# cnkuangshi/LightCTR

Hardware: NVIDIA B200
Metric: samples/sec (device-timed) FM train step on Criteo-shape (higher is better)
Workload: dtype f32

## Files before the change

lightctr_b200/csrc/capi.cu:

```cuda
#include <stdarg.h>
#include <stdlib.h>
#include <string.h>

#include <algorithm>
#include <vector>

#include "opt.cuh"

namespace lctr {
static thread_local std::string g_err;
void set_error(const char* fmt, ...) {
    char buf[1024];
    va_list ap;
    va_start(ap, fmt);
    vsnprintf(buf, sizeof(buf), fmt, ap);
    va_end(ap);
    g_err = buf;
}

template <typename T>
static int dalloc(T** p, size_t n) {
    *p = nullptr;
    if (n == 0) return 0;
    LCTR_CUDA(cudaMalloc((void**)p, n * sizeof(T)));
    return 0;
}
template <typename T>
static void dfree(T*& p) {
    if (p) cudaFree(p);
    p = nullptr;
}

static int slot_reserve(lctr_ctx* c, Slot& s, int64_t rows, int64_t nnz) {
    const size_t k = c->cfg.factor_cnt;
    if (rows > s.cap_rows) {
        int64_t cap = std::max<int64_t>(rows, s.cap_rows + s.cap_rows / 2);
        dfree(s.row_ptr); dfree(s.label); dfree(s.pred); dfree(s.sumvx); dfree(s.wide);
        if (dalloc(&s.row_ptr, (size_t)cap + 1)) return 1;
        if (dalloc(&s.label, (size_t)cap)) return 1;
        if (dalloc(&s.pred, (size_t)cap)) return 1;
        if (dalloc(&s.wide, (size_t)cap)) return 1;
        if (c->cfg.model != LCTR_MODEL_FFM) {
            if (dalloc(&s.sumvx, (size_t)cap * k)) return 1;
            LCTR_CUDA(cudaMemsetAsync(s.sumvx, 0, (size_t)cap * k * sizeof(float), c->stream));
        }
        s.cap_rows = cap;
    }
    if (nnz > s.cap_nnz) {
        int64_t cap = std::max<int64_t>(nnz, s.cap_nnz + s.cap_nnz / 2);
        dfree(s.fid); dfree(s.field); dfree(s.val);
        if (dalloc(&s.fid, (size_t)cap + 32)) return 1;
        if (dalloc(&s.field, (size_t)cap + 32)) return 1;
        if (dalloc(&s.val, (size_t)cap + 32)) return 1;
        s.cap_nnz = cap;
    }
    return 0;
}

__global__ void fill_value_kernel(float* p, size_t n, float v) {
    for (size_t i = (size_t)blockIdx.x * blockDim.x + threadIdx.x; i < n; i += (size_t)gridDim.x * blockDim.x) p[i] = v;
}

__global__ void label_to_float_kernel(const int32_t* in, float* out, int64_t n_arg, const int64_t* hdr) {
    const int64_t n = hdr ? hdr[0] : n_arg;
    int64_t i = (int64_t)blockIdx.x * blockDim.x + threadIdx.x;
    if (i < n) out[i] = (float)in[i];
}

__global__ void fill_params_kernel(float* __restrict__ W, float* __restrict__ V, size_t Fl, size_t rowlen, int rank,
                                   int world, unsigned long long seed, float scale) {
    const size_t n = Fl * rowlen;
    for (size_t i = (size_t)blockIdx.x * blockDim.x + threadIdx.x; i < n; i += (size_t)gridDim.x * blockDim.x) {
        const size_t l = i / rowlen, j = i % rowlen;
        const unsigned long long g = ((unsigned long long)(l * world + rank)) * rowlen + j;
        unsigned long long h = g * 0x9E3779B97F4A7C15ull + seed;
        h ^= h >> 33; h *= 0xff51afd7ed558ccdull; h ^= h >> 33; h *= 0xc4ceb9fe1a85ec53ull; h ^= h >> 33;
        const float u1 = ((unsigned)(h & 0xffffffu) + 1u) * (1.0f / 16777217.0f);
        const float u2 = (unsigned)((h >> 24) & 0xffffffu) * (1.0f / 16777216.0f);
        V[i] = scale * sqrtf(-2.0f * logf(u1)) * cosf(6.2831853f * u2);
        if (j == 0) W[l] = 0.f;
    }
}

static int build_csc(lctr_ctx* c, Slot& s, int64_t rows, int64_t nnz, const int64_t* row_ptr, const uint32_t* fid,
                     const float* val) {
    const int64_t block = c->cfg.csc_row_block ? (int64_t)c->cfg.csc_row_block : std::max<int64_t>(rows, 1);
    const int64_t nblocks = (rows + block - 1) / block;
    std::vector<int64_t> blk_seg_ptr(nblocks + 1, 0), seg_ptr;
    std::vector<uint32_t> seg_fid, ent_row((size_t)nnz);
    std::vector<float> ent_x(val ? (size_t)nnz : 0);
    seg_ptr.reserve((size_t)nnz / 4 + 16);
    seg_fid.reserve((size_t)nnz / 4 + 16);
    std::vector<uint32_t> cnt(c->F + 1, 0);
    std::vector<uint32_t> touched_list;
    int64_t out = 0;
    for (int64_t bi = 0; bi < nblocks; bi++) {
        const int64_t rb = bi * block, re = std::min(rows, rb + block);
        const int64_t eb = row_ptr[rb], ee = row_ptr[re];
        touched_list.clear();
        for (int64_t e = eb; e < ee; e++) {
            const uint32_t f = fid[e];
            if (f >= c->F) { set_error("upload_batch: fid %u >= feature_cnt %zu", f, c->F); return 1; }
            if (cnt[f]++ == 0) touched_list.push_back(f);
        }
        std::sort(touched_list.begin(), touched_list.end());
        for (uint32_t f : touched_list) {
            seg_fid.push_back(f);
            seg_ptr.push_back(out);
            const uint32_t n = cnt[f];
            cnt[f] = (uint32_t)(out - eb);
            out += n;
        }
        for (int64_t r = rb; r < re; r++)
            for (int64_t e = row_ptr[r]; e < row_ptr[r + 1]; e++) {
                const uint32_t f = fid[e];
                const int64_t pos = eb + cnt[f]++;
                ent_row[(size_t)pos] = (uint32_t)r;
                if (val) ent_x[(size_t)pos] = val[e];
            }
        for (uint32_t f : touched_list) cnt[f] = 0;
        blk_seg_ptr[bi + 1] = (int64_t)seg_fid.size();
    }
    seg_ptr.push_back(out);
    const int64_t nseg = (int64_t)seg_fid.size();
    if (nseg > s.cap_segs) {
        dfree(s.seg_ptr); dfree(s.seg_fid);
        if (dalloc(&s.seg_ptr, (size_t)nseg + 1) || dalloc(&s.seg_fid, (size_t)nseg + 1)) return 1;
        s.cap_segs = nseg;
    }
    if (nblocks > s.cap_blocks) {
        dfree(s.blk_seg_ptr);
        if (dalloc(&s.blk_seg_ptr, (size_t)nblocks + 1)) return 1;
        s.cap_blocks = nblocks;
    }
    if (nnz > s.cap_ent) {
        dfree(s.ent_row); dfree(s.ent_x);
        if (dalloc(&s.ent_row, (size_t)nnz + 32) || dalloc(&s.ent_x, (size_t)nnz + 32)) return 1;
        s.cap_ent = nnz;
    }
    LCTR_CUDA(cudaMemcpyAsync(s.seg_ptr, seg_ptr.data(), (size_t)(nseg + 1) * sizeof(int64_t), cudaMemcpyHostToDevice, c->stream));
    if (nseg) LCTR_CUDA(cudaMemcpyAsync(s.seg_fid, seg_fid.data(), (size_t)nseg * sizeof(uint32_t), cudaMemcpyHostToDevice, c->stream));
    LCTR_CUDA(cudaMemcpyAsync(s.blk_seg_ptr, blk_seg_ptr.data(), (size_t)(nblocks + 1) * sizeof(int64_t), cudaMemcpyHostToDevice, c->stream));
    if (nnz) {
        LCTR_CUDA(cudaMemcpyAsync(s.ent_row, ent_row.data(), (size_t)nnz * sizeof(uint32_t), cudaMemcpyHostToDevice, c->stream));
        if (val) LCTR_CUDA(cudaMemcpyAsync(s.ent_x, ent_x.data(), (size_t)nnz * sizeof(float), cudaMemcpyHostToDevice, c->stream));
    }
    LCTR_CUDA(cudaStreamSynchronize(c->stream));
    if (!s.h_blk_seg_ptr) s.h_blk_seg_ptr = new std::vector<int64_t>();
    *s.h_blk_seg_ptr = blk_seg_ptr;
    s.csc_block = block; s.n_blocks = nblocks; s.n_segs = nseg;
    return 0;
}
}

using namespace lctr;

extern "C" {

const char* lctr_last_error(void) { return g_err.c_str(); }
int lctr_abi_version(void) { return LCTR_ABI_VERSION; }

int lctr_create(const lctr_cfg* cfg, lctr_ctx** out) {
    LCTR_CHECK(cfg && out, "lctr_create: null argument");
    LCTR_CHECK(cfg->abi_version == LCTR_ABI_VERSION, "lctr_create: abi_version %u != %u", cfg->abi_version,
               LCTR_ABI_VERSION);
    LCTR_CHECK(cfg->model >= LCTR_MODEL_FM && cfg->model <= LCTR_MODEL_WND, "lctr_create: bad model %d", cfg->model);
    LCTR_CHECK(cfg->optimizer >= LCTR_OPT_ADAGRAD && cfg->optimizer <= LCTR_OPT_PS_DCASGDA, "lctr_create: bad optimizer %d",
               cfg->optimizer);
    LCTR_CHECK(cfg->feature_cnt > 0 && cfg->feature_cnt < (1ull << 32), "lctr_create: feature_cnt out of range");
    LCTR_CHECK(cfg->factor_cnt > 0, "lctr_create: factor_cnt must be > 0");
    LCTR_CHECK(cfg->model != LCTR_MODEL_FFM || cfg->field_cnt > 0, "lctr_create: FFM needs field_cnt > 0");
    if (cfg->model == LCTR_MODEL_WND) {
        LCTR_CHECK(cfg->field_cnt > 0 && cfg->field_cnt <= 2048, "lctr_create: Wide&Deep needs 0 < field_cnt <= 2048");
        LCTR_CHECK(cfg->deterministic == 0, "lctr_create: Wide&Deep uses the RED scatter (deterministic = 0)");
    }
    int ndev = 0;
    cudaError_t e = cudaGetDeviceCount(&ndev);
    if (e != cudaSuccess || ndev == 0) {
        set_error("lctr_create: no CUDA device available (%s); this library has no CPU fallback",
                  cudaGetErrorString(e));
        return 2;
    }
    LCTR_CHECK(cfg->device >= 0 && cfg->device < ndev, "lctr_create: device %d of %d", cfg->device, ndev);
    LCTR_CUDA(cudaSetDevice(cfg->device));
    lctr_ctx* c = new lctr_ctx();
    c->cfg = *cfg;
    if (c->cfg.ftrl_alpha == 0.f) {
        c->cfg.ftrl_alpha = 0.15f; c->cfg.ftrl_lambda1 = 1.0f; c->cfg.ftrl_beta = 1.0f; c->cfg.ftrl_lambda2 = 1.0f;
    }
    if (c->cfg.world <= 0) { c->cfg.world = 1; c->cfg.rank = 0; }
    c->F = cfg->feature_cnt;
    c->Fl = (c->F + (size_t)c->cfg.world - 1) / (size_t)c->cfg.world;
    LCTR_CHECK(c->cfg.world == 1 || !cfg->deterministic, "lctr_create: deterministic modes are single-GPU only");
    LCTR_CHECK(cfg->deterministic >= 0 && cfg->deterministic <= 2, "lctr_create: deterministic must be 0, 1 or 2");
    c->rowlen = cfg->model == LCTR_MODEL_FFM ? (size_t)cfg->field_cnt * cfg->factor_cnt : cfg->factor_cnt;
    cudaDeviceProp prop;
    LCTR_CUDA(cudaGetDeviceProperties(&prop, cfg->device));
    c->sm_count = prop.multiProcessorCount;
    LCTR_CUDA(cudaStreamCreateWithFlags(&c->stream, cudaStreamNonBlocking));
    const size_t FL = c->Fl;
    const size_t nv = FL * c->rowlen;
    const bool two = cfg->optimizer == LCTR_OPT_FTRL || cfg->optimizer == LCTR_OPT_ADAM || cfg->optimizer == LCTR_OPT_ADADELTA ||
                     cfg->optimizer == LCTR_OPT_PS_DCASGD || cfg->optimizer == LCTR_OPT_PS_DCASGDA;
    int rc = 0;
    rc |= dalloc(&c->W, FL); rc |= dalloc(&c->V, nv);
    rc |= dalloc(&c->gW, FL); rc |= dalloc(&c->gV, nv);
    rc |= dalloc(&c->s1W, FL); rc |= dalloc(&c->s1V, nv);
    if (two) { rc |= dalloc(&c->s2W, FL); rc |= dalloc(&c->s2V, nv); }
    rc |= dalloc(&c->touched, FL + 512);
    rc |= dalloc(&c->touch_list, FL + 32);
    rc |= dalloc(&c->n_touch, 1);
    rc |= dalloc(&c->apply_done, 1);
    rc |= dalloc(&c->stats, (size_t)2 * kStatRing);
    rc |= dalloc(&c->stat_partial, 2);
    rc |= dalloc(&c->stat_done, 1);
    if (rc) { lctr_destroy(c); return 1; }
    LCTR_CUDA(cudaMallocHost((void**)&c->h_stats, 2 * sizeof(double)));
    LCTR_CUDA(cudaMemsetAsync(c->W, 0, FL * sizeof(float), c->stream));
    LCTR_CUDA(cudaMemsetAsync(c->V, 0, nv * sizeof(float), c->stream));
    LCTR_CUDA(cudaMemsetAsync(c->gW, 0, FL * sizeof(float), c->stream));
    LCTR_CUDA(cudaMemsetAsync(c->gV, 0, nv * sizeof(float), c->stream));
    LCTR_CUDA(cudaMemsetAsync(c->s1W, 0, FL * sizeof(float), c->stream));
    LCTR_CUDA(cudaMemsetAsync(c->s1V, 0, nv * sizeof(float), c->stream));
    if (two) {
        LCTR_CUDA(cudaMemsetAsync(c->s2W, 0, FL * sizeof(float), c->stream));
        LCTR_CUDA(cudaMemsetAsync(c->s2V, 0, nv * sizeof(float), c->stream));
    }
    if (cfg->optimizer == LCTR_OPT_PS_ADAGRAD || cfg->optimizer == LCTR_OPT_PS_DCASGDA) {
        fill_value_kernel<<<c->sm_count * 4, 256, 0, c->stream>>>(c->s1W, FL, 1e-7f);
        fill_value_kernel<<<c->sm_count * 4, 256, 0, c->stream>>>(c->s1V, nv, 1e-7f);
    }
    LCTR_CUDA(cudaMemsetAsync(c->touched, 0, FL + 512, c->stream));
    if (c->cfg.world > 1) {
        if (dist_alloc(c)) { lctr_destroy(c); return 1; }
    } else {
        c->cW = c->W; c->cV = c->V; c->cgW = c->gW; c->cgV = c->gV;
    }
    LCTR_CUDA(cudaMemsetAsync(c->n_touch, 0, sizeof(unsigned int), c->stream));
    LCTR_CUDA(cudaMemsetAsync(c->apply_done, 0, sizeof(unsigned int), c->stream));
    LCTR_CUDA(cudaMemsetAsync(c->stats, 0, sizeof(double) * 2 * kStatRing, c->stream));
    LCTR_CUDA(cudaMemsetAsync(c->stat_partial, 0, sizeof(double) * 2, c->stream));
    LCTR_CUDA(cudaMemsetAsync(c->stat_done, 0, sizeof(unsigned int), c->stream));
    if (cfg->model == LCTR_MODEL_NFM || cfg->model == LCTR_MODEL_WND) {
        if (mlp_alloc(c)) { lctr_destroy(c); return 1; }
    }
    { const char* e = getenv("LCTR_CSC_IN_STEP"); c->csc_in_step = e && e[0] == '1'; }
    LCTR_CUDA(cudaStreamSynchronize(c->stream));
    *out = c;
    return 0;
}

int lctr_destroy(lctr_ctx* c) {
    if (!c) return 0;
    cudaSetDevice(c->cfg.device);
    if (c->stream) cudaStreamSynchronize(c->stream);
    dfree(c->W); dfree(c->V); dfree(c->gW); dfree(c->gV); dfree(c->s1W); dfree(c->s1V); dfree(c->s2W); dfree(c->s2V);
    dfree(c->touched); dfree(c->touch_list); dfree(c->n_touch); dfree(c->apply_done); dfree(c->stats); dfree(c->stat_partial); dfree(c->stat_done);
    for (auto& s : c->slots) {
        dfree(s.row_ptr); dfree(s.fid); dfree(s.field); dfree(s.val); dfree(s.label); dfree(s.pred); dfree(s.sumvx);
        dfree(s.wide);
        dfree(s.blk_seg_ptr); dfree(s.seg_ptr); dfree(s.seg_fid); dfree(s.ent_row); dfree(s.ent_x); dfree(s.ent_field);
        dfree(s.ent_slot); dfree(s.ent_pslot); dfree(s.hot_of); dfree(s.hot_slot); dfree(s.n_hot);
        dfree(s.uniq); dfree(s.n_uniq); dfree(s.short_list); dfree(s.long_list); dfree(s.csc_totals); dfree(s.csc_acc); dfree(s.csc_arrived);
        delete s.h_blk_seg_ptr; s.h_blk_seg_ptr = nullptr;
    }
    mlp_free(c);
    ffm_grouped_free(c);
    metrics_free(c);
    wnd_free(c);
    dist_free(c);
    fused_free(c);
    csc_scratch_free(c);
    if (c->h_stats) cudaFreeHost(c->h_stats);
    if (c->h_stat_ring) cudaFreeHost(c->h_stat_ring);
    for (int p = 0; p < kPipe; p++) {
        PipeGraph& g = c->pipe_graph[p];
        if (g.build) cudaGraphExecDestroy(g.build);
        if (g.step) cudaGraphExecDestroy(g.step);
        if (g.d_hdr) cudaFree(g.d_hdr); if (g.h_hdr) cudaFreeHost(g.h_hdr);
        if (g.d_opt) cudaFree(g.d_opt); if (g.h_opt) cudaFreeHost(g.h_opt);
        if (g.d_stat) cudaFree(g.d_stat); if (g.h_stat) cudaFreeHost(g.h_stat);
    }
    if (c->copy_stream) {
        for (int i = 0; i < kPipe; i++) { cudaEventDestroy(c->ev_copied[i]); cudaEventDestroy(c->ev_computed[i]); cudaEventDestroy(c->ev_h2d[i]); }
        if (c->build_stream) cudaStreamDestroy(c->build_stream);
        for (int i = 0; i < kStatRing; i++) cudaEventDestroy(c->ev_stat[i]);
        cudaStreamDestroy(c->copy_stream);
    }
    if (c->stream) cudaStreamDestroy(c->stream);
    delete c;
    return 0;
}

int lctr_sync(lctr_ctx* c) {
    LCTR_CHECK(c, "null ctx");
    LCTR_CUDA(cudaStreamSynchronize(c->stream));
    return 0;
}

int lctr_upload_params(lctr_ctx* c, const float* W, const float* V) {
    LCTR_CHECK(c, "null ctx");
    const int R = c->cfg.world, me = c->cfg.rank;
    if (R == 1) {
        if (W) LCTR_CUDA(cudaMemcpyAsync(c->W, W, c->F * sizeof(float), cudaMemcpyHostToDevice, c->stream));
        if (V) LCTR_CUDA(cudaMemcpyAsync(c->V, V, c->F * c->rowlen * sizeof(float), cudaMemcpyHostToDevice, c->stream));
    } else {
        std::vector<float> w, v;
        if (W) {
            w.assign(c->Fl, 0.f);
            for (size_t f = (size_t)me, l = 0; f < c->F; f += R, l++) w[l] = W[f];
            LCTR_CUDA(cudaMemcpyAsync(c->W, w.data(), c->Fl * sizeof(float), cudaMemcpyHostToDevice, c->stream));
        }
        if (V) {
            v.assign(c->Fl * c->rowlen, 0.f);
            for (size_t f = (size_t)me, l = 0; f < c->F; f += R, l++)
                memcpy(&v[l * c->rowlen], V + f * c->rowlen, c->rowlen * sizeof(float));
            LCTR_CUDA(cudaMemcpyAsync(c->V, v.data(), v.size() * sizeof(float), cudaMemcpyHostToDevice, c->stream));
        }
        LCTR_CUDA(cudaStreamSynchronize(c->stream));
        return 0;
    }
    LCTR_CUDA(cudaStreamSynchronize(c->stream));
    return 0;
}
int lctr_download_params(lctr_ctx* c, float* W, float* V) {
    LCTR_CHECK(c, "null ctx");
    const int R = c->cfg.world, me = c->cfg.rank;
    if (R == 1) {
        if (W) LCTR_CUDA(cudaMemcpyAsync(W, c->W, c->F * sizeof(float), cudaMemcpyDeviceToHost, c->stream));
        if (V) LCTR_CUDA(cudaMemcpyAsync(V, c->V, c->F * c->rowlen * sizeof(float), cudaMemcpyDeviceToHost, c->stream));
        LCTR_CUDA(cudaStreamSynchronize(c->stream));
        return 0;
    }
    std::vector<float> w(c->Fl), v(c->Fl * c->rowlen);
    LCTR_CUDA(cudaMemcpyAsync(w.data(), c->W, w.size() * sizeof(float), cudaMemcpyDeviceToHost, c->stream));
    LCTR_CUDA(cudaMemcpyAsync(v.data(), c->V, v.size() * sizeof(float), cudaMemcpyDeviceToHost, c->stream));
    LCTR_CUDA(cudaStreamSynchronize(c->stream));
    for (size_t f = (size_t)me, l = 0; f < c->F; f += R, l++) {
        if (W) W[f] = w[l];
        if (V) memcpy(V + f * c->rowlen, &v[l * c->rowlen], c->rowlen * sizeof(float));
    }
    return 0;
}
int lctr_fill_params(lctr_ctx* c, uint64_t seed, float scale) {
    LCTR_CHECK(c, "null ctx");
    fill_params_kernel<<<c->sm_count * 8, 256, 0, c->stream>>>(c->W, c->V, c->Fl, c->rowlen, c->cfg.rank, c->cfg.world,
                                                               (unsigned long long)seed, scale);
    c->launches++;
    LCTR_CUDA(cudaGetLastError());
    LCTR_CUDA(cudaStreamSynchronize(c->stream));
    return 0;
}
int lctr_download_opt_state(lctr_ctx* c, float* s1, float* s2) {
    LCTR_CHECK(c, "null ctx");
    LCTR_CHECK(c->cfg.world == 1, "optimizer-state transfer is single-GPU only");
    const size_t nv = c->F * c->rowlen;
    if (s1) {
        LCTR_CUDA(cudaMemcpyAsync(s1, c->s1W, c->F * sizeof(float), cudaMemcpyDeviceToHost, c->stream));
        LCTR_CUDA(cudaMemcpyAsync(s1 + c->F, c->s1V, nv * sizeof(float), cudaMemcpyDeviceToHost, c->stream));
    }
    if (s2 && c->s2W) {
        LCTR_CUDA(cudaMemcpyAsync(s2, c->s2W, c->F * sizeof(float), cudaMemcpyDeviceToHost, c->stream));
        LCTR_CUDA(cudaMemcpyAsync(s2 + c->F, c->s2V, nv * sizeof(float), cudaMemcpyDeviceToHost, c->stream));
    }
    LCTR_CUDA(cudaStreamSynchronize(c->stream));
    return 0;
}
int lctr_upload_opt_state(lctr_ctx* c, const float* s1, const float* s2) {
    LCTR_CHECK(c, "null ctx");
    LCTR_CHECK(c->cfg.world == 1, "optimizer-state transfer is single-GPU only (the state arrays are sharded by owner)");
    const size_t nv = c->F * c->rowlen;
    if (s1) {
        LCTR_CUDA(cudaMemcpyAsync(c->s1W, s1, c->F * sizeof(float), cudaMemcpyHostToDevice, c->stream));
        LCTR_CUDA(cudaMemcpyAsync(c->s1V, s1 + c->F, nv * sizeof(float), cudaMemcpyHostToDevice, c->stream));
    }
    if (s2 && c->s2W) {
        LCTR_CUDA(cudaMemcpyAsync(c->s2W, s2, c->F * sizeof(float), cudaMemcpyHostToDevice, c->stream));
        LCTR_CUDA(cudaMemcpyAsync(c->s2V, s2 + c->F, nv * sizeof(float), cudaMemcpyHostToDevice, c->stream));
    }
    LCTR_CUDA(cudaStreamSynchronize(c->stream));
    return 0;
}

static int upload_batch_on(lctr_ctx* c, cudaStream_t st, int slot, int64_t rows, int64_t nnz, const int64_t* row_ptr,
                           const uint32_t* fid, const uint16_t* field, const float* val, const int32_t* label) {
    LCTR_CHECK(c, "null ctx");
    LCTR_CHECK(slot >= 0 && slot < kNumSlots, "slot %d out of range", slot);
    LCTR_CHECK(rows >= 0 && nnz >= 0 && row_ptr && (nnz == 0 || fid) && (rows == 0 || label), "upload_batch: null input");
    LCTR_CHECK((c->cfg.model != LCTR_MODEL_FFM && c->cfg.model != LCTR_MODEL_WND) || field || nnz == 0,
               "upload_batch: FFM / Wide&Deep need the field array");
    Slot& s = c->slots[slot];
    if (rows > s.cap_rows || nnz > s.cap_nnz) {
        LCTR_CUDA(cudaStreamSynchronize(c->stream));
        if (slot_reserve(c, s, rows, nnz)) return 1;
        LCTR_CUDA(cudaStreamSynchronize(c->stream));
    }
    s.rows = rows; s.nnz = nnz;
    s.has_val = val != nullptr;
    s.has_field = field != nullptr;
    LCTR_CUDA(cudaMemcpyAsync(s.row_ptr, row_ptr, (size_t)(rows + 1) * sizeof(int64_t), cudaMemcpyHostToDevice, st));
    if (nnz) {
        LCTR_CUDA(cudaMemcpyAsync(s.fid, fid, (size_t)nnz * sizeof(uint32_t), cudaMemcpyHostToDevice, st));
        if (field) LCTR_CUDA(cudaMemcpyAsync(s.field, field, (size_t)nnz * sizeof(uint16_t), cudaMemcpyHostToDevice, st));
        if (val) LCTR_CUDA(cudaMemcpyAsync(s.val, val, (size_t)nnz * sizeof(float), cudaMemcpyHostToDevice, st));
    }
    const bool grouped = c->cfg.deterministic == 2 && rows > 0 && nnz > 0 && c->cfg.world == 1;
    int32_t* tmp = reinterpret_cast<int32_t*>(s.pred);
    if (rows) {
        LCTR_CUDA(cudaMemcpyAsync(tmp, label, (size_t)rows * sizeof(int32_t), cudaMemcpyHostToDevice, st));
        if (!grouped) {
            label_to_float_kernel<<<(unsigned)((rows + 255) / 256), 256, 0, st>>>(tmp, s.label, rows, nullptr);
            c->launches++;
            LCTR_CUDA(cudaGetLastError());
        }
    }
    s.fused_valid = false;
    if ((fused_supported(c) || c->cfg.world > 1) && rows > 0 && nnz > 0) {
        if (fused_reserve(c, s, nnz) || fused_build_slot(c, s, st, nullptr, rows, nnz)) return 1;
        if (c->cfg.world > 1 && dist_send_keys(c, s, slot, st)) return 1;
    }
    s.csc_block = 0;
    s.dev_csc = false;
    if (grouped) {
        LCTR_CHECK(csc_device_supported(c), "cfg.deterministic=2 (device-grouped backward) needs FM with k in {4,8,16,32} "
                                            "or FFM with k %% 4 == 0 and field_cnt * k <= 512");
        if (csc_build_device(c, s, st, tmp, nullptr, rows, nnz)) return 1;
    } else if (c->cfg.deterministic == 1 && c->cfg.model != LCTR_MODEL_FFM && rows > 0) {
        LCTR_CUDA(cudaStreamSynchronize(st));
        if (build_csc(c, s, rows, nnz, row_ptr, fid, val)) return 1;
    }
    return 0;
}

int lctr_upload_batch(lctr_ctx* c, int slot, int64_t rows, int64_t nnz, const int64_t* row_ptr, const uint32_t* fid,
                      const uint16_t* field, const float* val, const int32_t* label) {
    LCTR_CHECK(c, "null ctx");
    LCTR_CHECK(rows >= 0 && nnz >= 0 && row_ptr && (nnz == 0 || fid), "upload_batch: null input");
    LCTR_CHECK(row_ptr[0] == 0 && row_ptr[rows] == nnz, "upload_batch: row_ptr must run from 0 to nnz (%lld .. %lld, nnz %lld)",
               (long long)row_ptr[0], (long long)row_ptr[rows], (long long)nnz);
    for (int64_t r = 0; r < rows; r++)
        LCTR_CHECK(row_ptr[r] <= row_ptr[r + 1], "upload_batch: row_ptr decreases at row %lld", (long long)r);
    for (int64_t i = 0; i < nnz; i++)
        LCTR_CHECK(fid[i] < c->F, "upload_batch: fid %u at entry %lld >= feature_cnt %zu", fid[i], (long long)i, c->F);
    if ((c->cfg.model == LCTR_MODEL_FFM || c->cfg.model == LCTR_MODEL_WND) && field)
        for (int64_t i = 0; i < nnz; i++)
            LCTR_CHECK(field[i] < c->cfg.field_cnt, "upload_batch: field %u at entry %lld >= field_cnt %u", (unsigned)field[i],
                       (long long)i, c->cfg.field_cnt);
    return upload_batch_on(c, c->stream, slot, rows, nnz, row_ptr, fid, field, val, label);
}

static int read_stats(lctr_ctx* c, uint64_t step, float* loss_sum, float* acc_cnt) {
    if (!loss_sum && !acc_cnt) return 0;
    if (c->cfg.world > 1 && dist_check_overflow(c)) return 1;
    LCTR_CUDA(cudaMemcpyAsync(c->h_stats, c->stats + 2 * (step % kStatRing), 2 * sizeof(double), cudaMemcpyDeviceToHost,
                              c->stream));
    LCTR_CUDA(cudaStreamSynchronize(c->stream));
    if (loss_sum) *loss_sum = (float)c->h_stats[0];
    if (acc_cnt) *acc_cnt = (float)c->h_stats[1];
    return 0;
}

int lctr_train_step(lctr_ctx* c, int slot, int64_t rb, int64_t re, float* loss_sum, float* acc_cnt) {
    LCTR_CHECK(c, "null ctx");
    LCTR_CHECK(slot >= 0 && slot < kNumSlots, "slot %d out of range", slot);
    Slot& s = c->slots[slot];
    LCTR_CHECK(rb >= 0 && re <= s.rows && rb <= re, "train_step: rows [%lld,%lld) outside slot (%lld rows)",
               (long long)rb, (long long)re, (long long)s.rows);
    LCTR_CHECK(c->cfg.world == 1 || c->cfg.minibatch_size > 0,
               "train_step: multi-GPU contexts need cfg.minibatch_size = the GLOBAL batch (the updater's divisor)");
    const uint64_t step = c->step;
    int rc = 0;
    if (c->csc_in_step && c->cfg.deterministic == 2 && c->cfg.world == 1 && rb == 0 && re == s.rows && s.nnz > 0) {
        ProfScope prof(c, PROF_CSC_BUILD);
        if (csc_build_device(c, s, c->stream, nullptr, nullptr, s.rows, s.nnz)) return 1;
    }
    switch (c->cfg.model) {
        case LCTR_MODEL_FM:
            if (c->cfg.world > 1 && fused_kernels_ok(c))
                rc = dist_pre_step(c, s, slot, true) || launch_fm_fused(c, s, rb, re, true, nullptr, nullptr) ||
                     dist_post_step(c, s, slot, re - rb);
            else if (c->cfg.world > 1)
                rc = dist_pre_step(c, s, slot, false) || launch_fm_forward(c, s, rb, re, false, true) ||
                     launch_fm_backward(c, s, rb, re, false) || dist_post_step(c, s, slot, re - rb);
            else if (c->cfg.deterministic == 2)
                rc = launch_fm_forward(c, s, rb, re, false, true) || launch_fm_backward_devcsc(c, s, rb, re);
            else if (c->cfg.deterministic)
                rc = launch_fm_forward(c, s, rb, re, false, true) || launch_fm_backward_csc(c, s, rb, re, false);
            else if (s.fused_valid)
                rc = launch_fm_fused(c, s, rb, re, true, nullptr, nullptr) || launch_apply_compact(c, s, re - rb, nullptr, nullptr);
            else
                rc = launch_fm_forward(c, s, rb, re, false, true) || launch_fm_backward(c, s, rb, re, false) ||
                     launch_apply(c, re - rb);
            break;
        case LCTR_MODEL_FFM:
            if (c->cfg.world > 1)
                rc = dist_pre_step(c, s, slot, false) || launch_ffm_forward(c, s, rb, re, true) || dist_post_step(c, s, slot, re - rb);
            else if (c->cfg.deterministic == 2)
                rc = ffm_grouped_reserve(c, s.rows) || launch_ffm_forward_tiles(c, s, rb, re) ||
                     launch_ffm_backward_grouped(c, s, rb, re);
            else
                rc = launch_ffm_forward(c, s, rb, re, true) || launch_ffm_backward(c, s, rb, re) || launch_apply(c, re - rb);
            break;
        case LCTR_MODEL_WND:
            if (c->cfg.world > 1)
                rc = dist_pre_step(c, s, slot, false) || mlp_reserve(c, re - rb) || wnd_reserve(c, re - rb) ||
                     launch_wnd_forward(c, s, rb, re) || launch_nfm_mlp(c, s, rb, re, re - rb) || launch_wnd_backward(c, s, rb, re) ||
                     dist_post_step(c, s, slot, re - rb);
            else
                rc = mlp_reserve(c, re - rb) || wnd_reserve(c, re - rb) || launch_wnd_forward(c, s, rb, re) ||
                     launch_nfm_mlp(c, s, rb, re, re - rb) || launch_wnd_backward(c, s, rb, re) || launch_apply(c, re - rb);
            break;
        case LCTR_MODEL_NFM:
            if (fused_kernels_ok(c) && s.fused_valid) {
                const bool multi = c->cfg.world > 1;
                rc = (multi && dist_pre_step(c, s, slot, true)) || mlp_reserve(c, re - rb) || launch_nfm_forward_fused(c, s, rb, re) ||
                     launch_nfm_mlp(c, s, rb, re, re - rb) || launch_nfm_backward_fused(c, s, rb, re) ||
                     (multi ? dist_post_step(c, s, slot, re - rb) : launch_apply_compact(c, s, re - rb, nullptr, nullptr));
                break;
            }
            if (c->cfg.world > 1) {
                rc = dist_pre_step(c, s, slot, false) || mlp_reserve(c, re - rb) || launch_fm_forward(c, s, rb, re, true, false) ||
                     launch_nfm_mlp(c, s, rb, re, re - rb) || launch_fm_backward(c, s, rb, re, true) ||
                     dist_post_step(c, s, slot, re - rb);
                break;
            }
            rc = mlp_reserve(c, re - rb) || launch_fm_forward(c, s, rb, re, true, false) ||
                 launch_nfm_mlp(c, s, rb, re, re - rb);
            if (!rc) {
                if (c->cfg.deterministic == 1) rc = launch_fm_backward_csc(c, s, rb, re, true);
                else rc = launch_fm_backward(c, s, rb, re, true) || launch_apply(c, re - rb);
            }
            break;
    }
    if (rc) return 1;
    c->step++;
    return read_stats(c, step, loss_sum, acc_cnt);
}

int lctr_train_batch(lctr_ctx* c, int64_t rows, int64_t nnz, const int64_t* row_ptr, const uint32_t* fid,
                     const uint16_t* field, const float* val, const int32_t* label, float* loss_sum, float* acc_cnt) {
    if (lctr_upload_batch(c, 0, rows, nnz, row_ptr, fid, field, val, label)) return 1;
    return lctr_train_step(c, 0, 0, rows, loss_sum, acc_cnt);
}

static int pipe_init(lctr_ctx* c) {
    if (c->copy_stream) return 0;
    LCTR_CUDA(cudaStreamCreateWithFlags(&c->copy_stream, cudaStreamNonBlocking));
    LCTR_CUDA(cudaStreamCreateWithFlags(&c->build_stream, cudaStreamNonBlocking));
    for (int i = 0; i < kPipe; i++) {
        LCTR_CUDA(cudaEventCreateWithFlags(&c->ev_copied[i], cudaEventDisableTiming));
        LCTR_CUDA(cudaEventCreateWithFlags(&c->ev_computed[i], cudaEventDisableTiming));
        LCTR_CUDA(cudaEventCreateWithFlags(&c->ev_h2d[i], cudaEventDisableTiming));
    }
    for (int i = 0; i < kStatRing; i++) LCTR_CUDA(cudaEventCreateWithFlags(&c->ev_stat[i], cudaEventDisableTiming));
    LCTR_CUDA(cudaMallocHost((void**)&c->h_stat_ring, sizeof(double) * 2 * kStatRing));
    return 0;
}

static int pipe_graph_capture(lctr_ctx* c, int p, bool has_val) {
    PipeGraph& g = c->pipe_graph[p];
    Slot& s = c->slots[kNumSlots - kPipe + p];
    if (g.build) { cudaGraphExecDestroy(g.build); g.build = nullptr; }
    if (g.step) { cudaGraphExecDestroy(g.step); g.step = nullptr; }
    if (!g.d_hdr) {
        LCTR_CUDA(cudaMalloc((void**)&g.d_hdr, 2 * sizeof(int64_t)));
        LCTR_CUDA(cudaMallocHost((void**)&g.h_hdr, 2 * sizeof(int64_t)));
        LCTR_CUDA(cudaMalloc((void**)&g.d_opt, csc_opt_params_size()));
        LCTR_CUDA(cudaMallocHost((void**)&g.h_opt, csc_opt_params_size()));
        LCTR_CUDA(cudaMalloc((void**)&g.d_stat, 2 * sizeof(double)));
        LCTR_CUDA(cudaMallocHost((void**)&g.h_stat, 2 * sizeof(double)));
    }
    s.has_val = has_val;
    {
        OptParams* hp = reinterpret_cast<OptParams*>(g.h_opt);
        memset(hp, 0, csc_opt_params_size());
        hp->opt = c->cfg.optimizer;
    }
    cudaGraph_t graph;
    const bool fused = fused_supported(c);
    LCTR_CUDA(cudaStreamBeginCapture(c->copy_stream, cudaStreamCaptureModeThreadLocal));
    int rc = cudaMemcpyAsync(g.d_hdr, g.h_hdr, 2 * sizeof(int64_t), cudaMemcpyHostToDevice, c->copy_stream) != cudaSuccess;
    if (!rc) {
        if (fused) {
            label_to_float_kernel<<<(unsigned)((s.cap_rows + 255) / 256), 256, 0, c->copy_stream>>>(
                reinterpret_cast<int32_t*>(s.pred), s.label, s.cap_rows, g.d_hdr);
            c->launches++;
            rc = fused_build_slot(c, s, c->copy_stream, g.d_hdr, s.cap_rows, s.cap_nnz);
        } else {
            rc = csc_build_device(c, s, c->copy_stream, reinterpret_cast<int32_t*>(s.pred), g.d_hdr, s.cap_rows, s.cap_nnz);
        }
    }
    cudaError_t ce = cudaStreamEndCapture(c->copy_stream, &graph);
    if (rc || ce != cudaSuccess) { set_error("streamed pipeline: capture of the build graph failed (%s)", cudaGetErrorString(ce)); return 1; }
    LCTR_CUDA(cudaGraphInstantiate(&g.build, graph, 0));
    cudaGraphDestroy(graph);
    LCTR_CUDA(cudaStreamBeginCapture(c->stream, cudaStreamCaptureModeThreadLocal));
    rc = cudaMemcpyAsync(g.d_opt, g.h_opt, csc_opt_params_size(), cudaMemcpyHostToDevice, c->stream) != cudaSuccess;
    if (!rc) {
        if (fused)
            rc = launch_fm_fused(c, s, 0, s.cap_rows, true, g.d_hdr, g.d_stat) ||
                 launch_apply_compact(c, s, s.cap_rows, reinterpret_cast<const OptParams*>(g.h_opt),
                                      reinterpret_cast<const OptParams*>(g.d_opt));
        else
            rc = launch_fm_forward_ex(c, s, 0, s.cap_rows, false, true, g.d_hdr, g.d_stat) ||
                 launch_fm_backward_devcsc_ex(c, s, 0, s.cap_rows, reinterpret_cast<const OptParams*>(g.h_opt), g.d_opt);
    }
    if (!rc) rc = cudaMemcpyAsync(g.h_stat, g.d_stat, 2 * sizeof(double), cudaMemcpyDeviceToHost, c->stream) != cudaSuccess;
    ce = cudaStreamEndCapture(c->stream, &graph);
    if (rc || ce != cudaSuccess) { set_error("streamed pipeline: capture of the step graph failed (%s)", cudaGetErrorString(ce)); return 1; }
    LCTR_CUDA(cudaGraphInstantiate(&g.step, graph, 0));
    cudaGraphDestroy(graph);
    g.cap_rows = s.cap_rows; g.cap_nnz = s.cap_nnz; g.has_val = has_val;
    return 0;
}

static int train_batch_async_graph(lctr_ctx* c, int64_t rows, int64_t nnz, const int64_t* row_ptr, const uint32_t* fid,
                                   const float* val, const int32_t* label, uint64_t* ticket) {
    const int p = (int)(c->pipe_issued % kPipe);
    const int slot = kNumSlots - kPipe + p;
    Slot& s = c->slots[slot];
    PipeGraph& g = c->pipe_graph[p];
    if (rows > s.cap_rows || nnz > s.cap_nnz || !g.build || g.has_val != (val != nullptr) || g.cap_rows != s.cap_rows ||
        g.cap_nnz != s.cap_nnz) {
        LCTR_CUDA(cudaStreamSynchronize(c->stream));
        LCTR_CUDA(cudaStreamSynchronize(c->copy_stream));
        LCTR_CUDA(cudaStreamSynchronize(c->build_stream));
        if (rows > s.cap_rows || nnz > s.cap_nnz)
            if (slot_reserve(c, s, std::max(rows, s.cap_rows) + rows / 8 + 64, std::max(nnz, s.cap_nnz) + nnz / 8 + 1024)) return 1;
        if (fused_supported(c) ? fused_reserve(c, s, s.cap_nnz) : csc_reserve(c, s, s.cap_nnz)) return 1;
        LCTR_CUDA(cudaStreamSynchronize(c->stream));
        if (pipe_graph_capture(c, p, val != nullptr)) return 1;
    }
    s.rows = rows; s.nnz = nnz; s.has_val = val != nullptr; s.has_field = false;
    if (c->pipe_issued >= (uint64_t)kPipe) LCTR_CUDA(cudaStreamWaitEvent(c->copy_stream, c->ev_computed[p], 0));
    LCTR_CUDA(cudaMemcpyAsync(s.row_ptr, row_ptr, (size_t)(rows + 1) * sizeof(int64_t), cudaMemcpyHostToDevice, c->copy_stream));
    LCTR_CUDA(cudaMemcpyAsync(s.fid, fid, (size_t)nnz * sizeof(uint32_t), cudaMemcpyHostToDevice, c->copy_stream));
    if (val) LCTR_CUDA(cudaMemcpyAsync(s.val, val, (size_t)nnz * sizeof(float), cudaMemcpyHostToDevice, c->copy_stream));
    LCTR_CUDA(cudaMemcpyAsync(s.pred, label, (size_t)rows * sizeof(int32_t), cudaMemcpyHostToDevice, c->copy_stream));
    g.h_hdr[0] = rows; g.h_hdr[1] = nnz;
    LCTR_CUDA(cudaEventRecord(c->ev_h2d[p], c->copy_stream));
    LCTR_CUDA(cudaStreamWaitEvent(c->build_stream, c->ev_h2d[p], 0));
    LCTR_CUDA(cudaGraphLaunch(g.build, c->build_stream));
    LCTR_CUDA(cudaEventRecord(c->ev_copied[p], c->build_stream));
    LCTR_CUDA(cudaStreamWaitEvent(c->stream, c->ev_copied[p], 0));
    const bool fused = fused_supported(c);
    if (fused) fused_opt_params(c, rows, g.h_opt); else csc_opt_params(c, rows, g.h_opt);
    LCTR_CUDA(cudaGraphLaunch(g.step, c->stream));
    LCTR_CUDA(cudaEventRecord(c->ev_computed[p], c->stream));
    s.dev_csc = !fused;
    s.fused_valid = fused;
    c->launches += 8;
    g.ticket = c->step;
    *ticket = c->step++;
    c->pipe_issued++;
    return 0;
}

int lctr_train_batch_async(lctr_ctx* c, int64_t rows, int64_t nnz, const int64_t* row_ptr, const uint32_t* fid,
                           const uint16_t* field, const float* val, const int32_t* label, uint64_t* ticket) {
    LCTR_CHECK(c && ticket, "null argument");
    LCTR_CHECK(c->cfg.deterministic != 1, "streamed batches need cfg.deterministic 0 (RED scatter) or 2 (device grouping)");
    if (pipe_init(c)) return 1;
    LCTR_CHECK(c->pipe_issued - c->pipe_waited < (uint64_t)kPipe, "more than %d streamed batches outstanding: call lctr_wait first", kPipe);
    if ((c->cfg.deterministic == 2 || fused_supported(c)) && c->cfg.world == 1 && c->cfg.model == LCTR_MODEL_FM && !c->profiling &&
        rows > 0 && nnz > 0)
        return train_batch_async_graph(c, rows, nnz, row_ptr, fid, val, label, ticket);
    const int p = (int)(c->pipe_issued % kPipe);
    const int slot = kNumSlots - kPipe + p;
    if (c->pipe_issued >= (uint64_t)kPipe) LCTR_CUDA(cudaStreamWaitEvent(c->copy_stream, c->ev_computed[p], 0));
    if (c->pipe_issued >= 1) LCTR_CUDA(cudaStreamWaitEvent(c->copy_stream, c->ev_copied[(p + kPipe - 1) % kPipe], 0));
    if (upload_batch_on(c, c->copy_stream, slot, rows, nnz, row_ptr, fid, field, val, label)) return 1;
    LCTR_CUDA(cudaEventRecord(c->ev_copied[p], c->copy_stream));
    LCTR_CUDA(cudaStreamWaitEvent(c->stream, c->ev_copied[p], 0));
    const uint64_t step = c->step;
    if (lctr_train_step(c, slot, 0, rows, nullptr, nullptr)) return 1;
    LCTR_CUDA(cudaEventRecord(c->ev_computed[p], c->stream));
    const int ri = (int)(step % kStatRing);
    LCTR_CUDA(cudaMemcpyAsync(c->h_stat_ring + 2 * ri, c->stats + 2 * ri, 2 * sizeof(double), cudaMemcpyDeviceToHost, c->stream));
    LCTR_CUDA(cudaEventRecord(c->ev_stat[ri], c->stream));
    c->pipe_graph[p].ticket = ~0ull;
    *ticket = step;
    c->pipe_issued++;
    return 0;
}

int lctr_wait(lctr_ctx* c, uint64_t ticket, float* loss_sum, float* acc_cnt) {
    LCTR_CHECK(c && c->copy_stream, "lctr_wait: no streamed batch was issued");
    LCTR_CHECK(ticket < c->step && c->step - ticket <= (uint64_t)kStatRing, "lctr_wait: ticket %llu is not outstanding",
               (unsigned long long)ticket);
    for (int p = 0; p < kPipe; p++) {
        if (c->pipe_graph[p].build && c->pipe_graph[p].ticket == ticket) {
            LCTR_CUDA(cudaEventSynchronize(c->ev_computed[p]));
            if (loss_sum) *loss_sum = (float)c->pipe_graph[p].h_stat[0];
            if (acc_cnt) *acc_cnt = (float)c->pipe_graph[p].h_stat[1];
            if (c->pipe_waited < c->pipe_issued) c->pipe_waited++;
            return 0;
        }
    }
    const int ri = (int)(ticket % kStatRing);
    LCTR_CUDA(cudaEventSynchronize(c->ev_stat[ri]));
    if (loss_sum) *loss_sum = (float)c->h_stat_ring[2 * ri];
    if (acc_cnt) *acc_cnt = (float)c->h_stat_ring[2 * ri + 1];
    if (c->pipe_waited < c->pipe_issued) c->pipe_waited++;
    return 0;
}

int lctr_predict(lctr_ctx* c, int slot, int quirk_sumvx_slot, float* pctr) {
    LCTR_CHECK(c, "null ctx");
    LCTR_CHECK(slot >= 0 && slot < kNumSlots, "slot %d out of range", slot);
    Slot& s = c->slots[slot];
    int rc = 0;
    if (c->cfg.model == LCTR_MODEL_WND) {
        const float* out = nullptr;
        rc = (c->cfg.world > 1 && dist_pre_step(c, s, slot, false)) || mlp_reserve(c, s.rows) || wnd_reserve(c, s.rows) ||
             launch_wnd_forward(c, s, 0, s.rows) || mlp_forward_only(c, s.rows, &out) || launch_wnd_pred(c, s, out, 0, s.rows);
        if (rc) return 1;
        if (pctr) {
            LCTR_CUDA(cudaMemcpyAsync(pctr, s.pred, (size_t)s.rows * sizeof(float), cudaMemcpyDeviceToHost, c->stream));
            LCTR_CUDA(cudaStreamSynchronize(c->stream));
        }
        return 0;
    }
    LCTR_CHECK(c->cfg.world == 1, "lctr_predict: multi-GPU contexts keep sharded tables; download the parameters "
                                  "(lctr_download_params) into a single-GPU context to predict");
    if (c->cfg.model == LCTR_MODEL_FFM) {
        rc = c->cfg.deterministic == 1 ? launch_ffm_predict_inorder(c, s) : launch_ffm_forward(c, s, 0, s.rows, false);
    } else if (c->cfg.model == LCTR_MODEL_FM) {
        if (quirk_sumvx_slot >= 0) {
            LCTR_CHECK(quirk_sumvx_slot < kNumSlots, "quirk slot out of range");
            rc = launch_predict_quirk(c, s, c->slots[quirk_sumvx_slot]);
        } else {
            rc = fused_supported(c) ? launch_fm_forward_tree(c, s, 0, s.rows, false) : launch_fm_forward(c, s, 0, s.rows, false, false);
        }
    } else {
        set_error("lctr_predict: the reference ships no NFM predictor (main.cpp:230-233)");
        return 1;
    }
    if (rc) return 1;
    if (pctr) {
        LCTR_CUDA(cudaMemcpyAsync(pctr, s.pred, (size_t)s.rows * sizeof(float), cudaMemcpyDeviceToHost, c->stream));
        LCTR_CUDA(cudaStreamSynchronize(c->stream));
    }
    return 0;
}

int lctr_download_sumvx(lctr_ctx* c, int slot, float* out) {
    LCTR_CHECK(c && out, "null argument");
    LCTR_CHECK(slot >= 0 && slot < kNumSlots, "slot %d out of range", slot);
    Slot& s = c->slots[slot];
    LCTR_CHECK(s.sumvx, "model has no sumVX (FFM keeps it NULL, fm_predict.cpp:20)");
    LCTR_CUDA(cudaMemcpyAsync(out, s.sumvx, (size_t)s.rows * c->cfg.factor_cnt * sizeof(float), cudaMemcpyDeviceToHost,
                              c->stream));
    LCTR_CUDA(cudaStreamSynchronize(c->stream));
    return 0;
}
int lctr_download_pred(lctr_ctx* c, int slot, float* out) {
    LCTR_CHECK(c && out, "null argument");
    LCTR_CHECK(slot >= 0 && slot < kNumSlots, "slot %d out of range", slot);
    Slot& s = c->slots[slot];
    LCTR_CUDA(cudaMemcpyAsync(out, s.pred, (size_t)s.rows * sizeof(float), cudaMemcpyDeviceToHost, c->stream));
    LCTR_CUDA(cudaStreamSynchronize(c->stream));
    return 0;
}

int lctr_dense_grad_buffer(lctr_ctx* c, void** dev_ptr, size_t* n_floats) {
    LCTR_CHECK(c && dev_ptr && n_floats, "null argument");
    *dev_ptr = c->dense_grad;
    *n_floats = c->dense_grad_n;
    return 0;
}

int lctr_profile(lctr_ctx* c, int enable) {
    LCTR_CHECK(c, "null ctx");
    if (enable && !c->prof_ev) { c->prof_ev = new std::vector<cudaEvent_t>(); c->prof_id = new std::vector<int>(); }
    c->profiling = enable ? 1 : 0;
    return 0;
}
int lctr_profile_read(lctr_ctx* c, double* ms, int64_t* counts, int n, int reset) {
    LCTR_CHECK(c && ms && counts, "null argument");
    LCTR_CUDA(cudaStreamSynchronize(c->stream));
    if (c->prof_ev) {
        for (size_t i = 0; i < c->prof_id->size(); i++) {
            float t = 0.f;
            cudaEventElapsedTime(&t, (*c->prof_ev)[2 * i], (*c->prof_ev)[2 * i + 1]);
            const int id = (*c->prof_id)[i];
            if (id >= 0 && id < kNumProf) { c->prof_ms[id] += t; c->prof_cnt[id]++; }
            cudaEventDestroy((*c->prof_ev)[2 * i]); cudaEventDestroy((*c->prof_ev)[2 * i + 1]);
        }
        c->prof_ev->clear(); c->prof_id->clear();
    }
    for (int i = 0; i < n && i < kNumProf; i++) { ms[i] = c->prof_ms[i]; counts[i] = c->prof_cnt[i]; }
    if (reset) for (int i = 0; i < kNumProf; i++) { c->prof_ms[i] = 0; c->prof_cnt[i] = 0; }
    return 0;
}

int64_t lctr_launch_count(const lctr_ctx* c) { return c ? c->launches : 0; }
void* lctr_stream(lctr_ctx* c) { return c ? (void*)c->stream : nullptr; }

}
```

lightctr_b200/csrc/common.cuh:

```cuda
#pragma once
#include <cuda_runtime.h>
#include <stdint.h>
#include <stdio.h>
#include <string>
#include <vector>

#include "../../include/lightctr_b200.h"
#include "ref_expf.h"

namespace lctr {

void set_error(const char* fmt, ...);

#define LCTR_CUDA(call)                                                                         \
    do {                                                                                        \
        cudaError_t _e = (call);                                                                \
        if (_e != cudaSuccess) {                                                                \
            ::lctr::set_error("%s:%d: %s -> %s", __FILE__, __LINE__, #call, cudaGetErrorString(_e)); \
            return 1;                                                                           \
        }                                                                                       \
    } while (0)

#define LCTR_CHECK(cond, ...)                  \
    do {                                       \
        if (!(cond)) {                         \
            ::lctr::set_error(__VA_ARGS__);    \
            return 1;                          \
        }                                      \
    } while (0)

constexpr int kNumSlots = 8;
constexpr int kPipe = LCTR_PIPE_DEPTH;
constexpr int kNumProf = 16;
enum { PROF_FM_FWD = 0, PROF_FM_BWD_RED = 1, PROF_APPLY = 2, PROF_FFM_FUSED = 3, PROF_FM_BWD_CSC = 4, PROF_MLP = 5, PROF_DIST_MARK = 6, PROF_DIST_COMPACT = 7, PROF_DIST_PULL = 8, PROF_DIST_PUSH = 9, PROF_DIST_BAR0 = 10, PROF_DIST_MERGE = 11, PROF_DIST_BAR1 = 12, PROF_CSC_BUILD = 13, PROF_FM_FUSED = 14, PROF_APPLY_COMPACT = 15 };
constexpr int kStatRing = 64;
constexpr int kHotRep = 32;
constexpr int kHotMax = 2048;
constexpr uint32_t kHotBit = 0x80000000u;
constexpr unsigned kFull = 0xffffffffu;

struct Slot {
    int64_t rows = 0, nnz = 0, cap_rows = 0, cap_nnz = 0;
    int64_t* row_ptr = nullptr;
    uint32_t* fid = nullptr;
    uint16_t* field = nullptr;
    float* val = nullptr;
    float* label = nullptr;
    float* pred = nullptr;
    float* sumvx = nullptr;
    float* wide = nullptr;
    bool has_val = false, has_field = false;
    int64_t csc_block = 0;
    int64_t n_blocks = 0, n_segs = 0;
    int64_t* blk_seg_ptr = nullptr;
    int64_t* seg_ptr = nullptr;
    uint32_t* seg_fid = nullptr;
    uint32_t* ent_row = nullptr;
    float* ent_x = nullptr;
    uint16_t* ent_field = nullptr;
    std::vector<int64_t>* h_blk_seg_ptr = nullptr;
    int64_t cap_segs = 0, cap_blocks = 0, cap_ent = 0;
    bool dev_csc = false;
    uint32_t *short_list = nullptr, *long_list = nullptr;
    int64_t cap_long = 0;
    double* csc_acc = nullptr;
    unsigned int* csc_arrived = nullptr;
    unsigned int* csc_totals = nullptr;
    uint32_t* uniq = nullptr;
    unsigned int* n_uniq = nullptr;
    int64_t cap_uniq = 0;
    bool uniq_valid = false;
    uint32_t* ent_slot = nullptr;
    uint32_t* ent_pslot = nullptr;
    int64_t cap_ent_slot = 0;
    uint32_t *hot_of = nullptr, *hot_slot = nullptr;
    unsigned int* n_hot = nullptr;
    bool fused_valid = false;
};

struct PipeGraph {
    cudaGraphExec_t build = nullptr, step = nullptr;
    int64_t cap_rows = 0, cap_nnz = 0;
    bool has_val = false;
    int64_t *d_hdr = nullptr, *h_hdr = nullptr;
    void *d_opt = nullptr, *h_opt = nullptr;
    double *d_stat = nullptr, *h_stat = nullptr;
    uint64_t ticket = ~0ull;
};

struct MlpLayer {
    int in = 0, out = 0;
    float *w = nullptr, *b = nullptr, *mask = nullptr;
    float *dw = nullptr, *db = nullptr;
    float *acc_w = nullptr, *acc_b = nullptr;
    float* act = nullptr;
    float* delta = nullptr;
    void* w16 = nullptr;
    void* w16t = nullptr;
};

}

namespace lctr {
struct DistState;
struct OptParams;
struct FusedState {
    uint8_t* mark = nullptr;
    size_t T = 0;
    uint32_t* slot_of = nullptr;
    unsigned int* cnt = nullptr;
    size_t cnt_cap = 0;
    float* G = nullptr;
    size_t G_rows = 0;
    float* Ghot = nullptr;
    OptParams* d_opt = nullptr;
    int GS = 0;
};
}
struct lctr_ctx {
    lctr_cfg cfg;
    cudaStream_t stream = nullptr;
    size_t F = 0, rowlen = 0;
    size_t Fl = 0;
    float *W = nullptr, *V = nullptr, *gW = nullptr, *gV = nullptr;
    float *s1W = nullptr, *s1V = nullptr, *s2W = nullptr, *s2V = nullptr;
    uint8_t* touched = nullptr;
    float *cW = nullptr, *cV = nullptr, *cgW = nullptr, *cgV = nullptr;
    lctr::DistState* dist = nullptr;
    lctr::FusedState* fused = nullptr;
    size_t dist_rows = 0;
    uint32_t* touch_list = nullptr;
    unsigned int* n_touch = nullptr;
    unsigned int* apply_done = nullptr;
    double* stats = nullptr;
    double* stat_partial = nullptr;
    unsigned int* stat_done = nullptr;
    double* h_stats = nullptr;
    uint64_t step = 0;
    size_t adam_iter = 0;
    lctr::Slot slots[lctr::kNumSlots];
    int n_layers = 0;
    lctr::MlpLayer layers[LCTR_MAX_LAYERS + 1];
    float* dense_grad = nullptr;
    size_t dense_grad_n = 0;
    float *z = nullptr, *dz = nullptr;
    float* mlp_out = nullptr;
    size_t mlp_cap_rows = 0;
    int64_t mlp_fwd_rows = 0;
    uint32_t* wnd_src = nullptr;
    size_t wnd_cap_rows = 0;
    void* auc_scratch = nullptr;
    int csc_in_step = 0;
    float* ffm_T = nullptr;
    uint16_t* ffm_cnt = nullptr;
    size_t ffm_T_rows = 0;
    lctr_allreduce_fn dense_allreduce = nullptr;
    void* dense_allreduce_user = nullptr;
    int mlp_tm = 0;
    size_t mlp_smem = 0;
    int mlp_umma = 0;
    size_t mlp_umma_smem = 0;
    int mlp_has_mask = 0;
    int mlp_skip_update = 0;
    int sm_count = 148;
    int64_t launches = 0;
    const unsigned long long* apply_wait_flags = nullptr;
    int apply_wait_n = 0;
    unsigned long long apply_wait_epoch = 0;
    const float* fwd_quirk_sumvx = nullptr;
    int64_t fwd_quirk_rows = 0;
    void* csc_scratch = nullptr;
    int profiling = 0;
    std::vector<cudaEvent_t>* prof_ev = nullptr;
    std::vector<int>* prof_id = nullptr;
    double prof_ms[lctr::kNumProf] = {0};
    int64_t prof_cnt[lctr::kNumProf] = {0};
    cudaStream_t copy_stream = nullptr;
    cudaEvent_t ev_copied[lctr::kPipe] = {}, ev_computed[lctr::kPipe] = {};
    cudaStream_t build_stream = nullptr;
    cudaEvent_t ev_h2d[lctr::kPipe] = {};
    cudaEvent_t ev_stat[lctr::kStatRing] = {nullptr};
    double* h_stat_ring = nullptr;
    uint64_t pipe_issued = 0, pipe_waited = 0;
    lctr::PipeGraph pipe_graph[lctr::kPipe];
};

namespace lctr {

__device__ __forceinline__ float warp_sum(float v) {
#pragma unroll
    for (int o = 16; o > 0; o >>= 1) v += __shfl_xor_sync(kFull, v, o);
    return v;
}
__device__ __forceinline__ double warp_sum_d(double v) {
#pragma unroll
    for (int o = 16; o > 0; o >>= 1) v += __shfl_xor_sync(kFull, v, o);
    return v;
}
__device__ __forceinline__ void red_add_v4(float* addr, float4 v) {
    asm volatile("red.global.add.v4.f32 [%0], {%1, %2, %3, %4};" ::"l"(addr), "f"(v.x), "f"(v.y), "f"(v.z), "f"(v.w)
                 : "memory");
}
__device__ __forceinline__ void red_add_f32(float* addr, float v) {
    asm volatile("red.global.add.f32 [%0], %1;" ::"l"(addr), "f"(v) : "memory");
}
__device__ __forceinline__ float4 ldg_f4(const float* p) { return __ldg(reinterpret_cast<const float4*>(p)); }
__device__ __forceinline__ float4 ldg_f4_pinned(const float* p) {
    float4 v;
    asm volatile("ld.global.nc.v4.f32 {%0,%1,%2,%3}, [%4];" : "=f"(v.x), "=f"(v.y), "=f"(v.z), "=f"(v.w) : "l"(p));
    return v;
}
__device__ __forceinline__ float ldg_f32_pinned(const float* p) {
    float v;
    asm volatile("ld.global.nc.f32 %0, [%1];" : "=f"(v) : "l"(p));
    return v;
}

template <typename FX, typename FY>
__device__ __forceinline__ float avx_dot_seq(FX x, FY y, int n) {
    float result = 0.f;
    int i = 0;
    if (n > 7) {
        float d[8] = {0.f, 0.f, 0.f, 0.f, 0.f, 0.f, 0.f, 0.f};
        for (; i + 8 <= n; i += 8) {
#pragma unroll
            for (int l = 0; l < 8; l++) d[l] = d[l] + x(i + l) * y(i + l);
        }
        const float a0 = d[4] + d[0], a1 = d[5] + d[1], a2 = d[6] + d[2], a3 = d[7] + d[3];
        const float b0 = a0 + a2, b1 = a1 + a3;
        result = result + (b0 + b1);
    }
    for (; i < n; i++) result = result + x(i) * y(i);
    return result;
}

__device__ __forceinline__ float ref_sigmoid(float x) {
    if (x < -16.f) return 1e-7f;
    if (x > 16.f) return 0.99999988f;
    return 1.0f / (1.0f + lctr_ref_expf(-x));
}
__device__ __forceinline__ float ref_exp_any(float x) { return fabsf(x) < 87.f ? lctr_ref_expf(x) : expf(x); }
__device__ __forceinline__ void loss_terms(float p, float y, double& loss, double& correct) {
    loss = (y == 1.f) ? (double)(-logf(p)) : -log(1.0 - (double)p);
    correct = ((p > 0.5f && y == 1.f) || (p < 0.5f && y == 0.f)) ? 1.0 : 0.0;
}

__device__ __forceinline__ void publish_stats(double loss, double correct, double* partial, unsigned int* done,
                                               double* out_slot, bool accumulate_out) {
    __shared__ double sh[2][32];
    const int lane = threadIdx.x & 31, wid = threadIdx.x >> 5, nw = (blockDim.x + 31) >> 5;
    loss = warp_sum_d(loss);
    correct = warp_sum_d(correct);
    if (lane == 0) { sh[0][wid] = loss; sh[1][wid] = correct; }
    __syncthreads();
    if (wid == 0) {
        double a = lane < nw ? sh[0][lane] : 0.0, b = lane < nw ? sh[1][lane] : 0.0;
        a = warp_sum_d(a);
        b = warp_sum_d(b);
        if (lane == 0) {
            atomicAdd(&partial[0], a);
            atomicAdd(&partial[1], b);
            __threadfence();
            unsigned int prev = atomicAdd(done, 1u);
            if (prev == gridDim.x - 1) {
                __threadfence();
                double l = atomicAdd(&partial[0], 0.0), c = atomicAdd(&partial[1], 0.0);
                if (accumulate_out) { out_slot[0] += l; out_slot[1] += c; }
                else { out_slot[0] = l; out_slot[1] = c; }
                partial[0] = 0.0; partial[1] = 0.0;
                *done = 0u;
                __threadfence();
            }
        }
    }
}

struct ProfScope {
    lctr_ctx* c; int id; cudaEvent_t a = nullptr, b = nullptr;
    ProfScope(lctr_ctx* c_, int id_) : c(c_), id(id_) {
        if (!c->profiling) return;
        cudaEventCreate(&a); cudaEventCreate(&b);
        cudaEventRecord(a, c->stream);
    }
    ~ProfScope() {
        if (!a) return;
        cudaEventRecord(b, c->stream);
        c->prof_ev->push_back(a); c->prof_ev->push_back(b); c->prof_id->push_back(id);
    }
};
int launch_fm_forward(lctr_ctx* c, Slot& s, int64_t rb, int64_t re, bool nfm, bool stats);
int launch_fm_backward(lctr_ctx* c, Slot& s, int64_t rb, int64_t re, bool nfm);
int launch_ffm_forward(lctr_ctx* c, Slot& s, int64_t rb, int64_t re, bool stats);
int launch_ffm_backward(lctr_ctx* c, Slot& s, int64_t rb, int64_t re);
int launch_apply(lctr_ctx* c, int64_t rows_in_step);
int launch_fm_backward_csc(lctr_ctx* c, Slot& s, int64_t rb, int64_t re, bool nfm);
int csc_reserve(lctr_ctx* c, Slot& s, int64_t max_nnz);
int csc_build_device(lctr_ctx* c, Slot& s, cudaStream_t st, const int32_t* label_i32, const int64_t* hdr,
                     int64_t rows_cap, int64_t nnz_cap);
int launch_fm_backward_devcsc(lctr_ctx* c, Slot& s, int64_t rb, int64_t re);
struct OptParams;
int launch_fm_backward_devcsc_ex(lctr_ctx* c, Slot& s, int64_t rb, int64_t re, const OptParams* P_host, const void* dP);
void csc_opt_params(lctr_ctx* c, int64_t rows, void* out);
size_t csc_opt_params_size();
int launch_fm_forward_ex(lctr_ctx* c, Slot& s, int64_t rb, int64_t re, bool nfm, bool stats, const int64_t* hdr,
                         double* out_slot_override);
bool csc_device_supported(const lctr_ctx* c);
void csc_scratch_free(lctr_ctx* c);
int launch_predict_quirk(lctr_ctx* c, Slot& s, Slot& train);
bool fused_supported(const lctr_ctx* c);
bool fused_kernels_ok(const lctr_ctx* c);
void fused_free(lctr_ctx* c);
int fused_reserve(lctr_ctx* c, Slot& s, int64_t nnz);
int fused_build_slot(lctr_ctx* c, Slot& s, cudaStream_t st, const int64_t* hdr, int64_t rows_cap, int64_t nnz_cap);
void dist_wait_info(lctr_ctx* c, const unsigned long long** flags, int* n, unsigned long long* epoch);
int launch_fm_fused(lctr_ctx* c, Slot& s, int64_t rb, int64_t re, bool stats, const int64_t* hdr, double* out_slot_override);
int launch_fm_forward_tree(lctr_ctx* c, Slot& s, int64_t rb, int64_t re, bool stats);
int launch_nfm_forward_fused(lctr_ctx* c, Slot& s, int64_t rb, int64_t re);
int launch_nfm_backward_fused(lctr_ctx* c, Slot& s, int64_t rb, int64_t re);
int launch_apply_compact(lctr_ctx* c, Slot& s, int64_t rows_in_step, const OptParams* P_host, const OptParams* dP);
void fused_opt_params(lctr_ctx* c, int64_t rows, void* out);
void* fused_dev_opt(lctr_ctx* c);
int launch_ffm_predict_inorder(lctr_ctx* c, Slot& s);
int dist_alloc(lctr_ctx* c);
int dist_free(lctr_ctx* c);
int dist_send_keys(lctr_ctx* c, Slot& s, int slot, cudaStream_t st);
int dist_pre_step(lctr_ctx* c, Slot& s, int slot, bool in_kernel_wait);
int dist_post_step(lctr_ctx* c, Slot& s, int slot, int64_t rows_divisor);
int dist_check_overflow(lctr_ctx* c);
size_t dist_bytes(const lctr_ctx* c);
__global__ void compact_touched_kernel(uint8_t* touched, size_t F, uint32_t* list, unsigned int* n_list,
                                       const unsigned long long* wait_flags, int n_wait, unsigned long long wait_epoch);
int mlp_alloc(lctr_ctx* c);
int mlp_free(lctr_ctx* c);
int mlp_reserve(lctr_ctx* c, int64_t rows);
bool ffm_grouped_supported(const lctr_ctx* c);
int ffm_grouped_reserve(lctr_ctx* c, int64_t rows);
void ffm_grouped_free(lctr_ctx* c);
int launch_ffm_forward_tiles(lctr_ctx* c, Slot& s, int64_t rb, int64_t re);
int launch_ffm_backward_grouped(lctr_ctx* c, Slot& s, int64_t rb, int64_t re);
void metrics_free(lctr_ctx* c);
int wnd_reserve(lctr_ctx* c, int64_t rows);
void wnd_free(lctr_ctx* c);
int launch_wnd_forward(lctr_ctx* c, Slot& s, int64_t rb, int64_t re);
int launch_wnd_backward(lctr_ctx* c, Slot& s, int64_t rb, int64_t re);
int launch_wnd_pred(lctr_ctx* c, Slot& s, const float* mlp_out, int64_t rb, int64_t re);
int mlp_forward_only(lctr_ctx* c, int64_t rows, const float** out);
inline size_t mlp_in0(const lctr_cfg& cf) {
    return cf.model == LCTR_MODEL_WND ? (size_t)cf.field_cnt * cf.factor_cnt : (size_t)cf.factor_cnt;
}
int mlp_sync_dense_grad(lctr_ctx* c);
bool pdl_on();
void launch_slotmap_compact(lctr_ctx* c, uint8_t* mark, size_t T, uint32_t* uniq, unsigned int* n_uniq, cudaStream_t st);
int launch_ffm_warp(lctr_ctx* c, Slot& s, int64_t rb, int64_t re, bool stats);
int mlp_bf16_prepare(lctr_ctx* c);
int mlp_bf16_refresh(lctr_ctx* c, int layer);
int launch_nfm_mlp_bf16(lctr_ctx* c, Slot& s, int64_t rb, int64_t re, int64_t rows_divisor);
int launch_nfm_mlp(lctr_ctx* c, Slot& s, int64_t rb, int64_t re, int64_t rows_divisor);

}
```

lightctr_b200/csrc/fm_fused.cu:

```cuda
#include <algorithm>

#include "fm_fused.cuh"

namespace lctr {

bool fused_kernels_ok(const lctr_ctx* c) {
    const int k = (int)c->cfg.factor_cnt;
    return (c->cfg.model == LCTR_MODEL_FM || c->cfg.model == LCTR_MODEL_NFM) && c->cfg.deterministic == 0 &&
           (k == 4 || k == 8 || k == 16 || k == 32);
}
bool fused_supported(const lctr_ctx* c) { return c->cfg.world == 1 && fused_kernels_ok(c); }

void fused_free(lctr_ctx* c) {
    FusedState* f = c->fused;
    if (!f) return;
    cudaFree(f->mark); cudaFree(f->slot_of); cudaFree(f->cnt); cudaFree(f->G); cudaFree(f->Ghot); cudaFree(f->d_opt);
    delete f;
    c->fused = nullptr;
}

static int fused_init(lctr_ctx* c) {
    if (c->fused) return 0;
    FusedState* f = new FusedState();
    c->fused = f;
    f->T = mark_rows(c->F);
    f->GS = fused_kernels_ok(c) ? grad_stride((int)c->cfg.factor_cnt) : 0;
    LCTR_CUDA(cudaMalloc((void**)&f->mark, 128 * f->T + 512));
    LCTR_CUDA(cudaMemsetAsync(f->mark, 0, 128 * f->T + 512, c->stream));
    LCTR_CUDA(cudaMalloc((void**)&f->slot_of, c->F * sizeof(uint32_t)));
    if (f->GS) {
        LCTR_CUDA(cudaMalloc((void**)&f->Ghot, (size_t)kHotMax * kHotRep * f->GS * sizeof(float)));
        LCTR_CUDA(cudaMemsetAsync(f->Ghot, 0, (size_t)kHotMax * kHotRep * f->GS * sizeof(float), c->stream));
    }
    LCTR_CUDA(cudaMalloc((void**)&f->d_opt, sizeof(OptParams)));
    LCTR_CUDA(cudaStreamSynchronize(c->stream));
    return 0;
}

int fused_reserve(lctr_ctx* c, Slot& s, int64_t nnz) {
    if (fused_init(c)) return 1;
    FusedState* f = c->fused;
    const int64_t need_u = std::min<int64_t>(std::max<int64_t>(nnz, 1), (int64_t)c->F);
    if (nnz > s.cap_ent_slot) {
        LCTR_CUDA(cudaStreamSynchronize(c->stream));
        if (s.ent_slot) cudaFree(s.ent_slot);
        if (s.ent_pslot) cudaFree(s.ent_pslot);
        s.ent_pslot = nullptr;
        const int64_t cap = std::max<int64_t>(nnz, s.cap_ent_slot + s.cap_ent_slot / 2);
        LCTR_CUDA(cudaMalloc((void**)&s.ent_slot, (size_t)(cap + 64) * sizeof(uint32_t)));
        if (c->cfg.world > 1) LCTR_CUDA(cudaMalloc((void**)&s.ent_pslot, (size_t)(cap + 64) * sizeof(uint32_t)));
        s.cap_ent_slot = cap;
    }
    if (need_u > s.cap_uniq || !s.hot_of) {
        LCTR_CUDA(cudaStreamSynchronize(c->stream));
        if (s.uniq) cudaFree(s.uniq);
        if (s.hot_of) cudaFree(s.hot_of);
        const int64_t cap = std::min<int64_t>(std::max<int64_t>(need_u, s.cap_uniq + s.cap_uniq / 2), (int64_t)c->F);
        LCTR_CUDA(cudaMalloc((void**)&s.uniq, (size_t)(cap + 64) * sizeof(uint32_t)));
        LCTR_CUDA(cudaMalloc((void**)&s.hot_of, (size_t)(cap + 64) * sizeof(uint32_t)));
        if (!s.n_uniq) LCTR_CUDA(cudaMalloc((void**)&s.n_uniq, sizeof(unsigned int)));
        if (!s.n_hot) LCTR_CUDA(cudaMalloc((void**)&s.n_hot, sizeof(unsigned int)));
        if (!s.hot_slot) LCTR_CUDA(cudaMalloc((void**)&s.hot_slot, (size_t)kHotMax * sizeof(uint32_t)));
        s.cap_uniq = cap;
    }
    if ((size_t)s.cap_uniq > f->cnt_cap) {
        LCTR_CUDA(cudaStreamSynchronize(c->stream));
        if (c->copy_stream) LCTR_CUDA(cudaStreamSynchronize(c->copy_stream));
        if (f->cnt) cudaFree(f->cnt);
        LCTR_CUDA(cudaMalloc((void**)&f->cnt, (size_t)(s.cap_uniq + 64) * sizeof(unsigned int)));
        LCTR_CUDA(cudaMemset(f->cnt, 0, (size_t)(s.cap_uniq + 64) * sizeof(unsigned int)));
        f->cnt_cap = (size_t)s.cap_uniq;
    }
    const size_t g_rows = c->cfg.world > 1 ? c->dist_rows : (size_t)s.cap_uniq;
    if (f->GS && g_rows > f->G_rows) {
        LCTR_CUDA(cudaStreamSynchronize(c->stream));
        if (f->G) cudaFree(f->G);
        LCTR_CUDA(cudaMalloc((void**)&f->G, (g_rows + 64) * f->GS * sizeof(float)));
        LCTR_CUDA(cudaMemset(f->G, 0, (g_rows + 64) * f->GS * sizeof(float)));
        f->G_rows = g_rows;
    }
    return 0;
}

int fused_build_slot(lctr_ctx* c, Slot& s, cudaStream_t st, const int64_t* hdr, int64_t rows_cap, int64_t nnz_cap) {
    FusedState* f = c->fused;
    s.fused_valid = false;
    if (rows_cap <= 0 || nnz_cap <= 0) return 0;
    const int SM = c->sm_count;
    LCTR_CUDA(cudaMemsetAsync(s.n_uniq, 0, sizeof(unsigned int), st));
    LCTR_CUDA(cudaMemsetAsync(s.n_hot, 0, sizeof(unsigned int), st));
    const unsigned mkg = (unsigned)std::max<int64_t>(1, std::min<int64_t>((nnz_cap + 2047) / 2048, (int64_t)SM * 4));
    slotmap_mark_kernel<<<mkg, 256, 0, st>>>(s.fid, hdr, nnz_cap, f->mark, f->T);
    const size_t ntiles = (128 * f->T + 511) / 512;
    const unsigned cg = (unsigned)std::max<size_t>(1, std::min<size_t>((ntiles + 7) / 8, (size_t)SM * 8));
    slotmap_compact_kernel<<<cg, 256, 0, st>>>(f->mark, f->T, s.uniq, s.n_uniq, f->slot_of);
    const bool hot = f->GS != 0;
    if (hot) {
        const unsigned sg = (unsigned)std::min<int64_t>(((int64_t)kHotSampleRows * 128 + 255) / 256, (int64_t)SM * 8);
        slotmap_sample_kernel<<<sg, 256, 0, st>>>(s.row_ptr, s.fid, hdr, rows_cap, f->slot_of, f->cnt);
        slotmap_hot_kernel<<<SM * 2, 256, 0, st>>>(f->cnt, s.n_uniq, hdr, rows_cap, s.hot_of, s.hot_slot, s.n_hot);
        c->launches += 2;
    }
    const unsigned ag = (unsigned)std::max<int64_t>(1, std::min<int64_t>((nnz_cap + 255) / 256, (int64_t)SM * 8));
    slotmap_assign_kernel<<<ag, 256, 0, st>>>(s.fid, hdr, nnz_cap, f->slot_of, hot ? s.hot_of : nullptr, s.ent_slot,
                                              c->cfg.world > 1 ? s.ent_pslot : nullptr);
    c->launches += 3;
    LCTR_CUDA(cudaGetLastError());
    s.fused_valid = true;
    return 0;
}

void launch_slotmap_compact(lctr_ctx* c, uint8_t* mark, size_t T, uint32_t* uniq, unsigned int* n_uniq, cudaStream_t st) {
    const size_t ntiles = (128 * T + 511) / 512;
    const unsigned cg = (unsigned)std::max<size_t>(1, std::min<size_t>((ntiles + 7) / 8, (size_t)c->sm_count * 8));
    slotmap_compact_kernel<<<cg, 256, 0, st>>>(mark, T, uniq, n_uniq, nullptr);
}

bool pdl_on() {
    const char* e = getenv("LCTR_PDL");
    return !(e && atoi(e) == 0);
}

template <int K>
static void fused_go(lctr_ctx* c, Slot& s, int64_t rb, int64_t re, int stats, double* out_slot, const int64_t* hdr, int mode) {
    FusedState* f = c->fused;
    const unsigned grid = (unsigned)std::max<int64_t>(1, std::min<int64_t>((re - rb + 3) / 4, (int64_t)c->sm_count * 4));
    const bool multi = c->cfg.world > 1;
    const unsigned long long* wf = nullptr;
    int nw = 0;
    unsigned long long ep = 0;
    if (multi && mode != 3) dist_wait_info(c, &wf, &nw, &ep);
#define FUSED_ARGS s.row_ptr, multi ? s.ent_pslot : s.fid, s.ent_slot, s.val, s.label, c->cW, c->cV, s.pred, s.sumvx, nullptr, f->G, \
                   f->Ghot, f->GS, c->cfg.l2_reg, rb, re, hdr, c->stat_partial, c->stat_done, out_slot, stats, wf, nw, ep
#define FUSED_LAUNCH(HV)                                                                                                         \
    do {                                                                                                                         \
        if (mode == 1 && multi && pdl_on()) {   \
            cudaLaunchConfig_t cfg = {};                                                                                         \
            cfg.gridDim = dim3(grid); cfg.blockDim = dim3(128); cfg.stream = c->stream;                                          \
            cudaLaunchAttribute at[1];                                                                                           \
            at[0].id = cudaLaunchAttributeProgrammaticStreamSerialization;                                                       \
            at[0].val.programmaticStreamSerializationAllowed = 1;                                                                \
            cfg.attrs = at; cfg.numAttrs = 1;                                                                                    \
            cudaLaunchKernelEx(&cfg, fm_fused_kernel<K, HV, 1, false>, (const int64_t*)s.row_ptr, (const uint32_t*)s.ent_pslot,  \
                               (const uint32_t*)s.ent_slot, (const float*)s.val, (const float*)s.label, (const float*)c->cW,   \
                               (const float*)c->cV, s.pred, s.sumvx, (float*)nullptr, f->G, f->Ghot, f->GS, c->cfg.l2_reg, rb, re, hdr, \
                               c->stat_partial, c->stat_done, out_slot, stats, wf, nw, ep, (float*)nullptr, (float*)nullptr);    \
        } else if (mode == 1) fm_fused_kernel<K, HV, 1, false><<<grid, 128, 0, c->stream>>>(FUSED_ARGS);                         \
        else if (mode == 2) fm_fused_kernel<K, HV, 2, false><<<grid, 128, 0, c->stream>>>(FUSED_ARGS, c->z, s.wide);             \
        else {   \
            cudaLaunchConfig_t cfg = {};                                                                                         \
            cfg.gridDim = dim3(grid); cfg.blockDim = dim3(128); cfg.stream = c->stream;                                          \
            cudaLaunchAttribute at[1];                                                                                           \
            at[0].id = cudaLaunchAttributeProgrammaticStreamSerialization;                                                       \
            at[0].val.programmaticStreamSerializationAllowed = 1;                                                                \
            cfg.attrs = at; cfg.numAttrs = (!multi && pdl_on()) ? 1 : 0;                                                         \
            cudaLaunchKernelEx(&cfg, fm_fused_kernel<K, HV, 3, false>, (const int64_t*)s.row_ptr, (const uint32_t*)(multi ? s.ent_pslot : s.fid), \
                               (const uint32_t*)s.ent_slot, (const float*)s.val, (const float*)s.label, (const float*)c->cW,   \
                               (const float*)c->cV, s.pred, s.sumvx, (float*)nullptr, f->G, f->Ghot, f->GS, c->cfg.l2_reg, rb, re, hdr, \
                               c->stat_partial, c->stat_done, out_slot, stats, wf, nw, ep, c->dz, (float*)nullptr);              \
        }                                                                                                                        \
    } while (0)
    if (s.has_val) FUSED_LAUNCH(true); else FUSED_LAUNCH(false);
#undef FUSED_LAUNCH
#undef FUSED_ARGS
}

static int launch_fused_mode(lctr_ctx* c, Slot& s, int64_t rb, int64_t re, bool stats, const int64_t* hdr, double* out_slot_override,
                             int mode, int prof_id) {
    if (re - rb <= 0) return 0;
    LCTR_CHECK(s.fused_valid, "fused FM step on a slot without its slot map (uploaded before the context supported it?)");
    double* out_slot = out_slot_override ? out_slot_override : c->stats + 2 * (c->step % kStatRing);
    ProfScope prof(c, prof_id);
    switch ((int)c->cfg.factor_cnt) {
        case 4: fused_go<4>(c, s, rb, re, stats ? 1 : 0, out_slot, hdr, mode); break;
        case 8: fused_go<8>(c, s, rb, re, stats ? 1 : 0, out_slot, hdr, mode); break;
        case 16: fused_go<16>(c, s, rb, re, stats ? 1 : 0, out_slot, hdr, mode); break;
        default: fused_go<32>(c, s, rb, re, stats ? 1 : 0, out_slot, hdr, mode); break;
    }
    c->launches++;
    LCTR_CUDA(cudaGetLastError());
    return 0;
}

int launch_fm_fused(lctr_ctx* c, Slot& s, int64_t rb, int64_t re, bool stats, const int64_t* hdr, double* out_slot_override) {
    return launch_fused_mode(c, s, rb, re, stats, hdr, out_slot_override, 1, PROF_FM_FUSED);
}
int launch_nfm_forward_fused(lctr_ctx* c, Slot& s, int64_t rb, int64_t re) {
    return launch_fused_mode(c, s, rb, re, false, nullptr, nullptr, 2, PROF_FM_FWD);
}
int launch_nfm_backward_fused(lctr_ctx* c, Slot& s, int64_t rb, int64_t re) {
    return launch_fused_mode(c, s, rb, re, false, nullptr, nullptr, 3, PROF_FM_FUSED);
}

template <int K>
static void fwd_tree_go(lctr_ctx* c, Slot& s, int64_t rb, int64_t re, int stats, double* out_slot) {
    const int GS = grad_stride(K);
    const unsigned grid = (unsigned)std::max<int64_t>(1, std::min<int64_t>((re - rb + 3) / 4, (int64_t)c->sm_count * 4));
#define FWD_ARGS s.row_ptr, s.fid, s.fid, s.val, s.label, c->W, c->V, s.pred, s.sumvx, nullptr, nullptr, nullptr, GS, c->cfg.l2_reg, \
                 rb, re, nullptr, c->stat_partial, c->stat_done, out_slot, stats
    if (s.has_val) fm_fused_kernel<K, true, 0, true><<<grid, 128, 0, c->stream>>>(FWD_ARGS);
    else fm_fused_kernel<K, false, 0, true><<<grid, 128, 0, c->stream>>>(FWD_ARGS);
#undef FWD_ARGS
}
int launch_fm_forward_tree(lctr_ctx* c, Slot& s, int64_t rb, int64_t re, bool stats) {
    if (re - rb <= 0) return 0;
    double* out_slot = c->stats + 2 * (c->step % kStatRing);
    ProfScope prof(c, PROF_FM_FWD);
    switch ((int)c->cfg.factor_cnt) {
        case 4: fwd_tree_go<4>(c, s, rb, re, stats ? 1 : 0, out_slot); break;
        case 8: fwd_tree_go<8>(c, s, rb, re, stats ? 1 : 0, out_slot); break;
        case 16: fwd_tree_go<16>(c, s, rb, re, stats ? 1 : 0, out_slot); break;
        default: fwd_tree_go<32>(c, s, rb, re, stats ? 1 : 0, out_slot); break;
    }
    c->launches++;
    LCTR_CUDA(cudaGetLastError());
    return 0;
}

template <int K>
static void apply_go(lctr_ctx* c, Slot& s, const OptParams& P, const OptParams* P_dev) {
    FusedState* f = c->fused;
    const int main_blocks = c->sm_count * 3;
    const unsigned grid = (unsigned)(main_blocks + kHotMax / 8);
    const bool pdl_off = !pdl_on();
    cudaLaunchConfig_t cfg = {};
    cfg.gridDim = dim3(grid); cfg.blockDim = dim3(256); cfg.dynamicSmemBytes = 0; cfg.stream = c->stream;
    cudaLaunchAttribute attr[1];
    attr[0].id = cudaLaunchAttributeProgrammaticStreamSerialization;
    attr[0].val.programmaticStreamSerializationAllowed = 1;
    cfg.attrs = attr;
    cfg.numAttrs = (c->cfg.world == 1 && !pdl_off) ? 1 : 0;
#define AC_GO(OPTC)                                                                                                          \
    cudaLaunchKernelEx(&cfg, apply_compact_kernel<K, OPTC>, (const uint32_t*)s.uniq, (const unsigned int*)s.n_uniq, f->G,          \
                       (const uint32_t*)s.hot_of, (const uint32_t*)s.hot_slot, (const unsigned int*)s.n_hot, f->Ghot, f->GS,     \
                       main_blocks, c->W, c->V, c->s1W, c->s1V, c->s2W, c->s2V, P, P_dev)
    switch (P.opt) {
        case LCTR_OPT_ADAGRAD: AC_GO(LCTR_OPT_ADAGRAD); break;
        case LCTR_OPT_FTRL: AC_GO(LCTR_OPT_FTRL); break;
        case LCTR_OPT_ADAM: AC_GO(LCTR_OPT_ADAM); break;
        case LCTR_OPT_RMSPROP: AC_GO(LCTR_OPT_RMSPROP); break;
        case LCTR_OPT_ADADELTA: AC_GO(LCTR_OPT_ADADELTA); break;
        case LCTR_OPT_PS_SGD: AC_GO(LCTR_OPT_PS_SGD); break;
        case LCTR_OPT_PS_ADAGRAD: AC_GO(LCTR_OPT_PS_ADAGRAD); break;
        case LCTR_OPT_PS_DCASGD: AC_GO(LCTR_OPT_PS_DCASGD); break;
        default: AC_GO(LCTR_OPT_PS_DCASGDA); break;
    }
#undef AC_GO
}

int launch_apply_compact(lctr_ctx* c, Slot& s, int64_t rows_in_step, const OptParams* P_host, const OptParams* dP) {
    const OptParams P = P_host ? *P_host : make_opt_params(c, rows_in_step);
    ProfScope prof(c, PROF_APPLY_COMPACT);
    switch ((int)c->cfg.factor_cnt) {
        case 4: apply_go<4>(c, s, P, dP); break;
        case 8: apply_go<8>(c, s, P, dP); break;
        case 16: apply_go<16>(c, s, P, dP); break;
        default: apply_go<32>(c, s, P, dP); break;
    }
    c->launches++;
    LCTR_CUDA(cudaGetLastError());
    return 0;
}

void fused_opt_params(lctr_ctx* c, int64_t rows, void* out) { *reinterpret_cast<OptParams*>(out) = make_opt_params(c, rows); }
void* fused_dev_opt(lctr_ctx* c) { return c->fused ? (void*)c->fused->d_opt : nullptr; }

}
```

lightctr_b200/csrc/fm_fused.cuh:

```cuda
#pragma once
#include "opt.cuh"

namespace lctr {

constexpr int kHotSampleRows = 512;
__host__ __device__ constexpr int grad_stride(int k) { return k < 8 ? 8 : (k < 16 ? 16 : (k < 32 ? 32 : 64)); }

__device__ __forceinline__ uint32_t ldg_u32_pinned(const uint32_t* p) {
    uint32_t v;
    asm volatile("ld.global.nc.u32 %0, [%1];" : "=r"(v) : "l"(p));
    return v;
}

constexpr int kMarkTags = 2048;
__host__ __device__ inline size_t mark_rows(size_t F) { return (F + 127) / 128; }
__global__ void __launch_bounds__(256)
slotmap_mark_kernel(const uint32_t* __restrict__ fid, const int64_t* __restrict__ hdr, int64_t nnz_arg,
                    uint8_t* __restrict__ mark, size_t T) {
    __shared__ uint32_t tag[kMarkTags];
    const int64_t nnz = hdr ? hdr[1] : nnz_arg;
    for (int i = threadIdx.x; i < kMarkTags; i += blockDim.x) tag[i] = 0xffffffffu;
    __syncthreads();
    const int64_t per = (nnz + gridDim.x - 1) / gridDim.x;
    const int64_t b = (int64_t)blockIdx.x * per, e = min(nnz, b + per);
    for (int64_t i0 = b + threadIdx.x; i0 < e; i0 += 4 * blockDim.x) {
        uint32_t f[4];
#pragma unroll
        for (int u = 0; u < 4; u++) {
            const int64_t i = i0 + (int64_t)u * blockDim.x;
            f[u] = i < e ? ldg_u32_pinned(fid + i) : 0xffffffffu;
        }
#pragma unroll
        for (int u = 0; u < 4; u++) {
            if (f[u] == 0xffffffffu) continue;
            const uint32_t h = f[u] & (kMarkTags - 1);
            if (tag[h] != f[u]) {
                tag[h] = f[u];
                mark[(size_t)(f[u] & 127u) * T + (f[u] >> 7)] = 1;
            }
        }
    }
}

__global__ void __launch_bounds__(256)
slotmap_compact_kernel(uint8_t* __restrict__ mark, size_t T, uint32_t* __restrict__ uniq, unsigned int* __restrict__ n_uniq,
                       uint32_t* __restrict__ slot_of) {
    const size_t F = 128 * T;
    const int lane = threadIdx.x & 31;
    const size_t warp = (size_t)blockIdx.x * (blockDim.x >> 5) + (threadIdx.x >> 5);
    const size_t nwarps = (size_t)gridDim.x * (blockDim.x >> 5);
    const size_t ntiles = (F + 511) / 512;
    for (size_t tile = warp; tile < ntiles; tile += nwarps) {
        const size_t base = tile * 512 + (size_t)lane * 16;
        uint4 m = make_uint4(0, 0, 0, 0);
        if (base + 16 <= F) {
            m = *reinterpret_cast<const uint4*>(mark + base);
        } else if (base < F) {
            unsigned char tmp[16];
            for (int i = 0; i < 16; i++) tmp[i] = base + i < F ? mark[base + i] : 0;
            m = *reinterpret_cast<uint4*>(tmp);
        }
        const bool any = (m.x | m.y | m.z | m.w) != 0;
        if (!__any_sync(kFull, any)) continue;
        unsigned bits = 0;
        {
            const unsigned wv[4] = {m.x, m.y, m.z, m.w};
#pragma unroll
            for (int i = 0; i < 4; i++)
#pragma unroll
                for (int b = 0; b < 4; b++)
                    if ((wv[i] >> (8 * b)) & 0xffu) bits |= 1u << (i * 4 + b);
        }
        if (any) {
            if (base + 16 <= F) *reinterpret_cast<uint4*>(mark + base) = make_uint4(0, 0, 0, 0);
            else for (int i = 0; i < 16 && base + i < F; i++) mark[base + i] = 0;
        }
        const int mycnt = __popc(bits);
        int incl = mycnt;
#pragma unroll
        for (int o = 1; o < 32; o <<= 1) {
            const int t = __shfl_up_sync(kFull, incl, o);
            if (lane >= o) incl += t;
        }
        const int total = __shfl_sync(kFull, incl, 31);
        unsigned int gbase = 0;
        if (lane == 31) gbase = atomicAdd(n_uniq, (unsigned int)total);
        gbase = __shfl_sync(kFull, gbase, 31);
        unsigned int pos = gbase + (unsigned int)(incl - mycnt);
        while (bits) {
            const int bit = __ffs(bits) - 1;
            bits &= bits - 1;
            const size_t ps = base + bit;
            const uint32_t f = (uint32_t)(((ps % T) << 7) | (ps / T));
            uniq[pos] = f;
            if (slot_of) slot_of[f] = pos;
            pos++;
        }
    }
}

__global__ void __launch_bounds__(256)
slotmap_sample_kernel(const int64_t* __restrict__ row_ptr, const uint32_t* __restrict__ fid, const int64_t* __restrict__ hdr,
                      int64_t rows_arg, const uint32_t* __restrict__ slot_of, unsigned int* __restrict__ cnt) {
    const int64_t rows = hdr ? hdr[0] : rows_arg;
    const int64_t ns = row_ptr[rows < kHotSampleRows ? rows : kHotSampleRows];
    for (int64_t i = (int64_t)blockIdx.x * blockDim.x + threadIdx.x; i < ns; i += (int64_t)gridDim.x * blockDim.x)
        atomicAdd(&cnt[slot_of[fid[i]]], 1u);
}

__global__ void __launch_bounds__(256)
slotmap_hot_kernel(unsigned int* __restrict__ cnt, const unsigned int* __restrict__ n_uniq, const int64_t* __restrict__ hdr,
                   int64_t rows_arg, uint32_t* __restrict__ hot_of, uint32_t* __restrict__ hot_slot,
                   unsigned int* __restrict__ n_hot) {
    const int64_t rows = hdr ? hdr[0] : rows_arg;
    const int64_t srows = rows < kHotSampleRows ? rows : kHotSampleRows;
    const unsigned thr = (unsigned)max((int64_t)3, (128 * srows + rows - 1) / max(rows, (int64_t)1));
    const unsigned n = *n_uniq;
    const int lane = threadIdx.x & 31;
    for (unsigned b0 = (blockIdx.x * blockDim.x + threadIdx.x) - lane; b0 < n; b0 += gridDim.x * blockDim.x) {
        const unsigned i = b0 + lane;
        const bool hot = i < n && cnt[i] >= thr;
        const unsigned m = __ballot_sync(kFull, hot);
        unsigned base = 0;
        if (m && lane == 0) base = atomicAdd(n_hot, (unsigned)__popc(m));
        base = __shfl_sync(kFull, base, 0);
        if (i < n) {
            const unsigned h = base + (unsigned)__popc(m & ((1u << lane) - 1u));
            const bool take = hot && h < (unsigned)kHotMax;
            hot_of[i] = take ? h : 0xffffffffu;
            if (take) hot_slot[h] = i;
            cnt[i] = 0;
        }
    }
}

__global__ void __launch_bounds__(256)
slotmap_assign_kernel(const uint32_t* __restrict__ fid, const int64_t* __restrict__ hdr, int64_t nnz_arg,
                      const uint32_t* __restrict__ slot_of, const uint32_t* __restrict__ hot_of,
                      uint32_t* __restrict__ ent_slot, uint32_t* __restrict__ ent_pslot) {
    const int64_t nnz = hdr ? hdr[1] : nnz_arg;
    for (int64_t i = (int64_t)blockIdx.x * blockDim.x + threadIdx.x; i < nnz; i += (int64_t)gridDim.x * blockDim.x) {
        const uint32_t sl = slot_of[fid[i]];
        const uint32_t h = hot_of ? hot_of[sl] : 0xffffffffu;
        if (ent_slot) ent_slot[i] = h != 0xffffffffu ? (kHotBit | h) : sl;
        if (ent_pslot) ent_pslot[i] = sl;
    }
}

template <int K, bool HAS_VAL, int MODE, bool SAME_IDX, int MINB = 4>
__global__ void __launch_bounds__(128, MINB)
fm_fused_kernel(const int64_t* __restrict__ row_ptr, const uint32_t* __restrict__ pidx, const uint32_t* __restrict__ gidx,
                const float* __restrict__ val, const float* __restrict__ label, const float* __restrict__ W,
                const float* __restrict__ V, float* __restrict__ pred, float* __restrict__ sumvx, float* __restrict__ dvec,
                float* __restrict__ G, float* __restrict__ Ghot, int GS, float l2, int64_t rb, int64_t re_arg,
                const int64_t* __restrict__ hdr, double* partial, unsigned int* done, double* out_slot, int do_stats,
                const unsigned long long* wait_flags = nullptr, int n_wait = 0, unsigned long long wait_epoch = 0,
                float* __restrict__ zbuf = nullptr ,
                float* __restrict__ wide = nullptr ) {
    constexpr bool FWD = MODE != 3, BWD = MODE == 1 || MODE == 3, NFM = MODE >= 2;
    static_assert(K % 4 == 0 && K <= 32 && (K / 4 & (K / 4 - 1)) == 0, "fused FM step: K in {4, 8, 16, 32}");
    cudaTriggerProgrammaticLaunchCompletion();
    if (wait_flags) {
        if (threadIdx.x < n_wait) {
            const volatile unsigned long long* f = wait_flags + threadIdx.x;
            while (*f < wait_epoch) __nanosleep(40);
            __threadfence();
        }
        __syncthreads();
    }
    constexpr int LPR = K / 4;
    constexpr int GR = 32 / LPR;
    constexpr int NPASS = K <= 8 ? 8 : (K == 16 ? 4 : 2);
    const int lane = threadIdx.x & 31;
    const int q = lane % LPR, g = lane / LPR;
    const int64_t re = hdr ? hdr[0] : re_arg;
    const int64_t NW = (int64_t)gridDim.x * (blockDim.x >> 5);
    const int64_t gwarp = (int64_t)blockIdx.x * (blockDim.x >> 5) + (threadIdx.x >> 5);
    const int rep = (int)(gwarp & (kHotRep - 1));
    double loss = 0.0, correct = 0.0;

    for (int64_t c0 = rb + gwarp; c0 < re; c0 += 32 * NW) {
        const int64_t myr = c0 + (int64_t)lane * NW;
        long long mb = 0;
        int mn = 0;
        if (myr < re) {
            mb = row_ptr[myr];
            mn = (int)(row_ptr[myr + 1] - mb);
        }
        const int cnt = (int)min((int64_t)32, (re - c0 + NW - 1) / NW);
        uint32_t pf[NPASS], gs[NPASS];
        float xs[NPASS];
        {
            const long long b = __shfl_sync(kFull, mb, 0);
            const int n = __shfl_sync(kFull, mn, 0);
#pragma unroll
            for (int p = 0; p < NPASS; p++) {
                const int i = p * 32 + lane;
                const bool ok = i < n;
                pf[p] = ok ? ldg_u32_pinned(pidx + b + i) : 0u;
                gs[p] = SAME_IDX ? pf[p] : ((ok && BWD) ? ldg_u32_pinned(gidx + b + i) : 0u);
                xs[p] = ok ? (HAS_VAL ? ldg_f32_pinned(val + b + i) : 1.f) : 0.f;
            }
        }
        cudaGridDependencySynchronize();
        for (int t = 0; t < cnt; t++) {
            const int64_t r = c0 + (int64_t)t * NW;
            const long long b = __shfl_sync(kFull, mb, t);
            const int n = __shfl_sync(kFull, mn, t);
            float4 v[NPASS][LPR];
            float ws[NPASS];
#pragma unroll
            for (int p = 0; p < NPASS; p++) {
                if (p * 32 < n) {
                    ws[p] = ldg_f32_pinned(W + pf[p]);
#pragma unroll
                    for (int it = 0; it < LPR; it++) {
                        const uint32_t fj = __shfl_sync(kFull, pf[p], it * GR + g);
                        v[p][it] = ldg_f4_pinned(V + (size_t)fj * K + 4 * q);
                    }
                } else {
                    ws[p] = 0.f;
#pragma unroll
                    for (int it = 0; it < LPR; it++) v[p][it] = make_float4(0.f, 0.f, 0.f, 0.f);
                }
            }
            uint32_t npf[NPASS], ngs[NPASS];
            float nxs[NPASS];
            {
                const int tn = t + 1 < cnt ? t + 1 : t;
                const long long bn = __shfl_sync(kFull, mb, tn);
                const int nn_raw = __shfl_sync(kFull, mn, tn);
                const int nn = t + 1 < cnt ? nn_raw : 0;
#pragma unroll
                for (int p = 0; p < NPASS; p++) {
                    const int i = p * 32 + lane;
                    const bool ok = i < nn;
                    npf[p] = ok ? ldg_u32_pinned(pidx + bn + i) : 0u;
                    ngs[p] = SAME_IDX ? npf[p] : ((ok && BWD) ? ldg_u32_pinned(gidx + bn + i) : 0u);
                    nxs[p] = ok ? (HAS_VAL ? ldg_f32_pinned(val + bn + i) : 1.f) : 0.f;
                }
            }
            float4 s = make_float4(0.f, 0.f, 0.f, 0.f);
            float4 sqv = make_float4(0.f, 0.f, 0.f, 0.f);
            float sq = 0.f, wsum = 0.f;
            if (FWD) {
#pragma unroll
                for (int p = 0; p < NPASS; p++) {
                    if (p * 32 < n) {
                        wsum = __fmaf_rn(ws[p], HAS_VAL ? xs[p] : (p * 32 + lane < n ? 1.f : 0.f), wsum);
#pragma unroll
                        for (int it = 0; it < LPR; it++) {
                            const float xj = HAS_VAL ? __shfl_sync(kFull, xs[p], it * GR + g)
                                                     : (p * 32 + it * GR + g < n ? 1.f : 0.f);
                            const float4 tt = make_float4(v[p][it].x * xj, v[p][it].y * xj, v[p][it].z * xj, v[p][it].w * xj);
                            s.x += tt.x; s.y += tt.y; s.z += tt.z; s.w += tt.w;
                            if (NFM) {
                                sqv.x = __fmaf_rn(tt.x, tt.x, sqv.x); sqv.y = __fmaf_rn(tt.y, tt.y, sqv.y);
                                sqv.z = __fmaf_rn(tt.z, tt.z, sqv.z); sqv.w = __fmaf_rn(tt.w, tt.w, sqv.w);
                            } else {
                                sq = __fmaf_rn(tt.x, tt.x, sq); sq = __fmaf_rn(tt.y, tt.y, sq);
                                sq = __fmaf_rn(tt.z, tt.z, sq); sq = __fmaf_rn(tt.w, tt.w, sq);
                            }
                        }
                    }
                }
                for (int base = NPASS * 32; base < n; base += 32) {
                    const int i = base + lane;
                    const bool ok = i < n;
                    const uint32_t f = ok ? __ldg(pidx + b + i) : 0u;
                    const float x = ok ? (HAS_VAL ? __ldg(val + b + i) : 1.f) : 0.f;
                    wsum = __fmaf_rn(__ldg(W + f), x, wsum);
                    float4 vv[LPR];
#pragma unroll
                    for (int it = 0; it < LPR; it++) {
                        const uint32_t fj = __shfl_sync(kFull, f, it * GR + g);
                        vv[it] = ldg_f4(V + (size_t)fj * K + 4 * q);
                    }
#pragma unroll
                    for (int it = 0; it < LPR; it++) {
                        const float xj = __shfl_sync(kFull, x, it * GR + g);
                        const float4 tt = make_float4(vv[it].x * xj, vv[it].y * xj, vv[it].z * xj, vv[it].w * xj);
                        s.x += tt.x; s.y += tt.y; s.z += tt.z; s.w += tt.w;
                        if (NFM) {
                            sqv.x = __fmaf_rn(tt.x, tt.x, sqv.x); sqv.y = __fmaf_rn(tt.y, tt.y, sqv.y);
                            sqv.z = __fmaf_rn(tt.z, tt.z, sqv.z); sqv.w = __fmaf_rn(tt.w, tt.w, sqv.w);
                        } else {
                            sq = __fmaf_rn(tt.x, tt.x, sq); sq = __fmaf_rn(tt.y, tt.y, sq);
                            sq = __fmaf_rn(tt.z, tt.z, sq); sq = __fmaf_rn(tt.w, tt.w, sq);
                        }
                    }
                }
#pragma unroll
                for (int o = LPR; o < 32; o <<= 1) {
                    s.x += __shfl_xor_sync(kFull, s.x, o); s.y += __shfl_xor_sync(kFull, s.y, o);
                    s.z += __shfl_xor_sync(kFull, s.z, o); s.w += __shfl_xor_sync(kFull, s.w, o);
                    if (NFM) {
                        sqv.x += __shfl_xor_sync(kFull, sqv.x, o); sqv.y += __shfl_xor_sync(kFull, sqv.y, o);
                        sqv.z += __shfl_xor_sync(kFull, sqv.z, o); sqv.w += __shfl_xor_sync(kFull, sqv.w, o);
                    }
                }
                wsum = warp_sum(wsum);
                if (lane < LPR) *reinterpret_cast<float4*>(sumvx + (size_t)r * K + 4 * q) = s;
            }
            float d = 0.f;
            float4 dz4 = make_float4(0.f, 0.f, 0.f, 0.f);
            if (!NFM) {
                sq = warp_sum(sq);
                float dot = s.x * s.x + s.y * s.y + s.z * s.z + s.w * s.w;
#pragma unroll
                for (int o = 1; o < LPR; o <<= 1) dot += __shfl_xor_sync(kFull, dot, o);
                const float fm = wsum - 0.5f * sq + 0.5f * dot;
                const float pr = ref_sigmoid(fm);
                const float y = __ldg(label + r);
                d = pr - y;
                if (lane == 0) {
                    pred[r] = pr;
                    if (dvec) dvec[r] = d;
                    if (do_stats) {
                        double l1, c1;
                        loss_terms(pr, y, l1, c1);
                        loss += l1;
                        correct += c1;
                    }
                }
            } else if (MODE == 2) {
                if (lane < LPR) {
                    const float4 z4 = make_float4(0.5f * (s.x * s.x - sqv.x), 0.5f * (s.y * s.y - sqv.y),
                                                  0.5f * (s.z * s.z - sqv.z), 0.5f * (s.w * s.w - sqv.w));
                    *reinterpret_cast<float4*>(zbuf + (size_t)(r - rb) * K + 4 * q) = z4;
                }
                if (lane == 0) wide[r] = wsum;
            } else {
                s = __ldg(reinterpret_cast<const float4*>(sumvx + (size_t)r * K + 4 * q));
                dz4 = __ldg(reinterpret_cast<const float4*>(zbuf + (size_t)(r - rb) * K + 4 * q));
                d = __ldg(pred + r) - __ldg(label + r);
            }
            if (BWD) {
#pragma unroll
                for (int p = 0; p < NPASS; p++) {
                    if (p * 32 < n) {
#pragma unroll
                        for (int it = 0; it < LPR; it++) {
                            const int j = it * GR + g;
                            const float xj = HAS_VAL ? __shfl_sync(kFull, xs[p], j) : 1.f;
                            const float wj = __shfl_sync(kFull, ws[p], j);
                            const uint32_t sj = __shfl_sync(kFull, gs[p], j);
                            if (p * 32 + j < n) {
                                const float gw = __fmaf_rn(d, xj, l2 * wj);
                                const float4 vv = v[p][it];
                                const float4 mu = NFM ? make_float4(dz4.x * xj, dz4.y * xj, dz4.z * xj, dz4.w * xj) : make_float4(gw, gw, gw, gw);
                                float4 gv;
                                gv.x = __fmaf_rn(__fmaf_rn(-xj, vv.x, s.x), mu.x, l2 * vv.x);
                                gv.y = __fmaf_rn(__fmaf_rn(-xj, vv.y, s.y), mu.y, l2 * vv.y);
                                gv.z = __fmaf_rn(__fmaf_rn(-xj, vv.z, s.z), mu.z, l2 * vv.z);
                                gv.w = __fmaf_rn(__fmaf_rn(-xj, vv.w, s.w), mu.w, l2 * vv.w);
                                float* dst = (sj & kHotBit) ? Ghot + ((size_t)(sj & ~kHotBit) * kHotRep + rep) * GS
                                                            : G + (size_t)sj * GS;
                                red_add_v4(dst + 4 * q, gv);
                                if (q == 0) red_add_f32(dst + K, gw);
                            }
                        }
                    }
                }
                for (int base = NPASS * 32; base < n; base += 32) {
                    const int i = base + lane;
                    const bool ok = i < n;
                    const uint32_t f = ok ? __ldg(pidx + b + i) : 0u;
                    const uint32_t sl = ok ? __ldg(gidx + b + i) : 0u;
                    const float x = ok ? (HAS_VAL ? __ldg(val + b + i) : 1.f) : 0.f;
                    const float w = __ldg(W + f);
#pragma unroll
                    for (int it = 0; it < LPR; it++) {
                        const int j = it * GR + g;
                        const uint32_t fj = __shfl_sync(kFull, f, j);
                        const uint32_t sj = __shfl_sync(kFull, sl, j);
                        const float xj = __shfl_sync(kFull, x, j);
                        const float wj = __shfl_sync(kFull, w, j);
                        if (base + j < n) {
                            const float4 vv = ldg_f4(V + (size_t)fj * K + 4 * q);
                            const float gw = __fmaf_rn(d, xj, l2 * wj);
                            const float4 mu = NFM ? make_float4(dz4.x * xj, dz4.y * xj, dz4.z * xj, dz4.w * xj) : make_float4(gw, gw, gw, gw);
                            float4 gv;
                            gv.x = __fmaf_rn(__fmaf_rn(-xj, vv.x, s.x), mu.x, l2 * vv.x);
                            gv.y = __fmaf_rn(__fmaf_rn(-xj, vv.y, s.y), mu.y, l2 * vv.y);
                            gv.z = __fmaf_rn(__fmaf_rn(-xj, vv.z, s.z), mu.z, l2 * vv.z);
                            gv.w = __fmaf_rn(__fmaf_rn(-xj, vv.w, s.w), mu.w, l2 * vv.w);
                            float* dst = (sj & kHotBit) ? Ghot + ((size_t)(sj & ~kHotBit) * kHotRep + rep) * GS
                                                        : G + (size_t)sj * GS;
                            red_add_v4(dst + 4 * q, gv);
                            if (q == 0) red_add_f32(dst + K, gw);
                        }
                    }
                }
            }
#pragma unroll
            for (int p = 0; p < NPASS; p++) { pf[p] = npf[p]; gs[p] = ngs[p]; xs[p] = nxs[p]; }
        }
    }
    if (do_stats) publish_stats(loss, correct, partial, done, out_slot, false);
}

template <int K, int OPT>
__global__ void __launch_bounds__(256, 3)
apply_compact_kernel(const uint32_t* __restrict__ uniq, const unsigned int* __restrict__ n_uniq, float* __restrict__ G,
                     const uint32_t* __restrict__ hot_of, const uint32_t* __restrict__ hot_slot,
                     const unsigned int* __restrict__ n_hot, float* __restrict__ Ghot, int GS, int main_blocks,
                     float* __restrict__ W, float* __restrict__ V, float* __restrict__ s1W, float* __restrict__ s1V,
                     float* __restrict__ s2W, float* __restrict__ s2V, OptParams P_in, const OptParams* __restrict__ P_dev) {
    constexpr int LPR = K / 4, GR = 32 / LPR, U = 2;
    OptParams P = P_dev ? *P_dev : P_in;
    P.opt = OPT;
    constexpr bool two = OPT == LCTR_OPT_FTRL || OPT == LCTR_OPT_ADAM || OPT == LCTR_OPT_ADADELTA || OPT == LCTR_OPT_PS_DCASGD ||
                         OPT == LCTR_OPT_PS_DCASGDA;
    const int lane = threadIdx.x & 31;
    if ((int)blockIdx.x >= main_blocks) {
        const unsigned hwarp = (blockIdx.x - main_blocks) * (blockDim.x >> 5) + (threadIdx.x >> 5);
        const unsigned nhw = (gridDim.x - main_blocks) * (blockDim.x >> 5);
        const unsigned nh = min(*n_hot, (unsigned)kHotMax);
        for (unsigned h = hwarp; h < nh; h += nhw) {
            const uint32_t slot = __ldg(hot_slot + h);
            const uint32_t f = __ldg(uniq + slot);
            float* tile = Ghot + (size_t)h * kHotRep * GS;
#pragma unroll
            for (int c0 = 0; c0 < K + 1; c0 += 32) {
                const int ncol = GS < 32 ? GS : 32;
                const int col = c0 + lane % ncol;
                const int grp = lane / ncol, ngrp = 32 / ncol;
                float wv = 0.f, av = 0.f, bv = 0.f;
                const bool mine = grp == 0 && col <= K;
                const size_t o = col < K ? (size_t)f * K + col : (size_t)f;
                if (mine) {
                    wv = col < K ? V[o] : W[o];
                    av = col < K ? s1V[o] : s1W[o];
                    if (two) bv = col < K ? s2V[o] : s2W[o];
                }
                cudaGridDependencySynchronize();
                float t[kHotRep];
#pragma unroll
                for (int i = 0; i < kHotRep; i++)
                    t[i] = (i < kHotRep / ngrp) ? __ldcg(tile + (size_t)(grp + i * ngrp) * GS + col) : 0.f;
                float sum = 0.f;
#pragma unroll
                for (int i = 0; i < kHotRep; i++) {
                    sum += t[i];
                    if (i < kHotRep / ngrp) tile[(size_t)(grp + i * ngrp) * GS + col] = 0.f;
                }
                for (int o2 = ncol; o2 < 32; o2 <<= 1) sum += __shfl_xor_sync(kFull, sum, o2);
                if (mine) {
                    update_one(P, col < K ? P.corrV : P.corrW, wv, sum, av, bv);
                    if (col < K) { V[o] = wv; s1V[o] = av; if (two) s2V[o] = bv; }
                    else { W[o] = wv; s1W[o] = av; if (two) s2W[o] = bv; }
                }
            }
        }
        cudaGridDependencySynchronize();
        return;
    }
    const unsigned warp = blockIdx.x * (blockDim.x >> 5) + (threadIdx.x >> 5);
    const unsigned nwarps = (unsigned)main_blocks * (blockDim.x >> 5);
    const int q = lane % LPR, g = lane / LPR;
    const unsigned total = *n_uniq;
    for (unsigned b0 = warp * (GR * U); b0 < total; b0 += nwarps * (GR * U)) {
        uint32_t f[U];
        bool ok[U];
        float4 g4[U], v4[U], a4[U], b4[U];
        float gw[U], w[U], a[U], bb[U];
#pragma unroll
        for (int u = 0; u < U; u++) {
            const unsigned idx = b0 + u * GR + g;
            ok[u] = idx < total && !(hot_of && __ldg(hot_of + idx) != 0xffffffffu);
            f[u] = ok[u] ? __ldg(uniq + idx) : 0u;
            g4[u] = v4[u] = a4[u] = b4[u] = make_float4(0.f, 0.f, 0.f, 0.f);
            gw[u] = w[u] = a[u] = bb[u] = 0.f;
            if (ok[u]) {
                const size_t o = (size_t)f[u] * K + 4 * q;
                v4[u] = *reinterpret_cast<const float4*>(V + o);
                a4[u] = *reinterpret_cast<const float4*>(s1V + o);
                if (two) b4[u] = *reinterpret_cast<const float4*>(s2V + o);
                if (q == 0) {
                    w[u] = W[f[u]]; a[u] = s1W[f[u]];
                    if (two) bb[u] = s2W[f[u]];
                }
            }
        }
        cudaGridDependencySynchronize();
#pragma unroll
        for (int u = 0; u < U; u++) {
            if (ok[u]) {
                const float* grow = G + (size_t)(b0 + u * GR + g) * GS;
                g4[u] = *reinterpret_cast<const float4*>(grow + 4 * q);
                if (q == 0) gw[u] = grow[K];
            }
        }
#pragma unroll
        for (int u = 0; u < U; u++) {
            if (!ok[u]) continue;
            const unsigned idx = b0 + u * GR + g;
            float* grow = G + (size_t)idx * GS;
            const size_t o = (size_t)f[u] * K + 4 * q;
            update_one(P, P.corrV, v4[u].x, g4[u].x, a4[u].x, b4[u].x);
            update_one(P, P.corrV, v4[u].y, g4[u].y, a4[u].y, b4[u].y);
            update_one(P, P.corrV, v4[u].z, g4[u].z, a4[u].z, b4[u].z);
            update_one(P, P.corrV, v4[u].w, g4[u].w, a4[u].w, b4[u].w);
            *reinterpret_cast<float4*>(V + o) = v4[u];
            *reinterpret_cast<float4*>(s1V + o) = a4[u];
            if (two) *reinterpret_cast<float4*>(s2V + o) = b4[u];
            *reinterpret_cast<float4*>(grow + 4 * q) = make_float4(0.f, 0.f, 0.f, 0.f);
            if (q == 0) {
                update_one(P, P.corrW, w[u], gw[u], a[u], bb[u]);
                W[f[u]] = w[u]; s1W[f[u]] = a[u];
                if (two) s2W[f[u]] = bb[u];
                grow[K] = 0.f;
            }
        }
    }
    cudaGridDependencySynchronize();
}

}
```

Baseline: 114.4 million.

## Fuse FM fused step and compact optimizer apply into one cooperative kernel

Replaces the two-kernel single-GPU FM fused path (forward/backward kernel followed by apply_compact) with one cooperative-launch kernel. It prefetches the parameters and optimizer state of unique rows at the start, runs forward/backward, then does a grid-wide sync before the compact optimizer update. This removes a launch and the handoff between kernels, and lets the parameter loads overlap with compute. In exchange the grid is capped at occupancy-limited residency, and the whole grid must wait at a barrier. The apply kernel is also refactored onto a shared updater with an occupancy-sized grid.

```diff
diff --git a/lightctr_b200/csrc/capi.cu b/lightctr_b200/csrc/capi.cu
--- a/lightctr_b200/csrc/capi.cu
+++ b/lightctr_b200/csrc/capi.cu
@@ -487,7 +487,7 @@
             else if (c->cfg.deterministic)
                 rc = launch_fm_forward(c, s, rb, re, false, true) || launch_fm_backward_csc(c, s, rb, re, false);
             else if (s.fused_valid)
-                rc = launch_fm_fused(c, s, rb, re, true, nullptr, nullptr) || launch_apply_compact(c, s, re - rb, nullptr, nullptr);
+                rc = launch_fm_step(c, s, rb, re, nullptr, nullptr, nullptr, nullptr);
             else
                 rc = launch_fm_forward(c, s, rb, re, false, true) || launch_fm_backward(c, s, rb, re, false) ||
                      launch_apply(c, re - rb);
@@ -515,7 +515,7 @@
                 const bool multi = c->cfg.world > 1;
                 rc = (multi && dist_pre_step(c, s, slot, true)) || mlp_reserve(c, re - rb) || launch_nfm_forward_fused(c, s, rb, re) ||
                      launch_nfm_mlp(c, s, rb, re, re - rb) || launch_nfm_backward_fused(c, s, rb, re) ||
-                     (multi ? dist_post_step(c, s, slot, re - rb) : launch_apply_compact(c, s, re - rb, nullptr, nullptr));
+                     (multi ? dist_post_step(c, s, slot, re - rb) : launch_apply_compact(c, s, re - rb));
                 break;
             }
             if (c->cfg.world > 1) {
@@ -598,9 +598,8 @@
     rc = cudaMemcpyAsync(g.d_opt, g.h_opt, csc_opt_params_size(), cudaMemcpyHostToDevice, c->stream) != cudaSuccess;
     if (!rc) {
         if (fused)
-            rc = launch_fm_fused(c, s, 0, s.cap_rows, true, g.d_hdr, g.d_stat) ||
-                 launch_apply_compact(c, s, s.cap_rows, reinterpret_cast<const OptParams*>(g.h_opt),
-                                      reinterpret_cast<const OptParams*>(g.d_opt));
+            rc = launch_fm_step(c, s, 0, s.cap_rows, g.d_hdr, g.d_stat, reinterpret_cast<const OptParams*>(g.h_opt),
+                                reinterpret_cast<const OptParams*>(g.d_opt));
         else
             rc = launch_fm_forward_ex(c, s, 0, s.cap_rows, false, true, g.d_hdr, g.d_stat) ||
                  launch_fm_backward_devcsc_ex(c, s, 0, s.cap_rows, reinterpret_cast<const OptParams*>(g.h_opt), g.d_opt);
@@ -649,7 +648,7 @@
     LCTR_CUDA(cudaEventRecord(c->ev_computed[p], c->stream));
     s.dev_csc = !fused;
     s.fused_valid = fused;
-    c->launches += 8;
+    c->launches += fused ? 7 : 8;
     g.ticket = c->step;
     *ticket = c->step++;
     c->pipe_issued++;
diff --git a/lightctr_b200/csrc/common.cuh b/lightctr_b200/csrc/common.cuh
--- a/lightctr_b200/csrc/common.cuh
+++ b/lightctr_b200/csrc/common.cuh
@@ -115,6 +115,8 @@
     float* Ghot = nullptr;
     OptParams* d_opt = nullptr;
     int GS = 0;
+    int step_grid[2] = {0, 0};
+    int apply_grid = 0;
 };
 }
 struct lctr_ctx {
@@ -314,10 +316,12 @@
 int fused_build_slot(lctr_ctx* c, Slot& s, cudaStream_t st, const int64_t* hdr, int64_t rows_cap, int64_t nnz_cap);
 void dist_wait_info(lctr_ctx* c, const unsigned long long** flags, int* n, unsigned long long* epoch);
 int launch_fm_fused(lctr_ctx* c, Slot& s, int64_t rb, int64_t re, bool stats, const int64_t* hdr, double* out_slot_override);
+int launch_fm_step(lctr_ctx* c, Slot& s, int64_t rb, int64_t re, const int64_t* hdr, double* out_slot_override,
+                   const OptParams* P_host, const OptParams* dP);
 int launch_fm_forward_tree(lctr_ctx* c, Slot& s, int64_t rb, int64_t re, bool stats);
 int launch_nfm_forward_fused(lctr_ctx* c, Slot& s, int64_t rb, int64_t re);
 int launch_nfm_backward_fused(lctr_ctx* c, Slot& s, int64_t rb, int64_t re);
-int launch_apply_compact(lctr_ctx* c, Slot& s, int64_t rows_in_step, const OptParams* P_host, const OptParams* dP);
+int launch_apply_compact(lctr_ctx* c, Slot& s, int64_t rows_in_step);
 void fused_opt_params(lctr_ctx* c, int64_t rows, void* out);
 void* fused_dev_opt(lctr_ctx* c);
 int launch_ffm_predict_inorder(lctr_ctx* c, Slot& s);
diff --git a/lightctr_b200/csrc/fm_fused.cu b/lightctr_b200/csrc/fm_fused.cu
--- a/lightctr_b200/csrc/fm_fused.cu
+++ b/lightctr_b200/csrc/fm_fused.cu
@@ -142,9 +142,10 @@
             at[0].val.programmaticStreamSerializationAllowed = 1;                                                                \
             cfg.attrs = at; cfg.numAttrs = 1;                                                                                    \
             cudaLaunchKernelEx(&cfg, fm_fused_kernel<K, HV, 1, false>, (const int64_t*)s.row_ptr, (const uint32_t*)s.ent_pslot,  \
-                               (const uint32_t*)s.ent_slot, (const float*)s.val, (const float*)s.label, (const float*)c->cW,   \
-                               (const float*)c->cV, s.pred, s.sumvx, (float*)nullptr, f->G, f->Ghot, f->GS, c->cfg.l2_reg, rb, re, hdr, \
-                               c->stat_partial, c->stat_done, out_slot, stats, wf, nw, ep, (float*)nullptr, (float*)nullptr);    \
+                               (const uint32_t*)s.ent_slot, (const float*)s.val, (const float*)s.label, c->cW, c->cV, s.pred,  \
+                               s.sumvx, (float*)nullptr, f->G, f->Ghot, f->GS, c->cfg.l2_reg, rb, re, hdr,                      \
+                               c->stat_partial, c->stat_done, out_slot, stats, wf, nw, ep, (float*)nullptr, (float*)nullptr,     \
+                               CompactUpd{});                                                                            \
         } else if (mode == 1) fm_fused_kernel<K, HV, 1, false><<<grid, 128, 0, c->stream>>>(FUSED_ARGS);                         \
         else if (mode == 2) fm_fused_kernel<K, HV, 2, false><<<grid, 128, 0, c->stream>>>(FUSED_ARGS, c->z, s.wide);             \
         else {   \
@@ -155,9 +156,9 @@
             at[0].val.programmaticStreamSerializationAllowed = 1;                                                                \
             cfg.attrs = at; cfg.numAttrs = (!multi && pdl_on()) ? 1 : 0;                                                         \
             cudaLaunchKernelEx(&cfg, fm_fused_kernel<K, HV, 3, false>, (const int64_t*)s.row_ptr, (const uint32_t*)(multi ? s.ent_pslot : s.fid), \
-                               (const uint32_t*)s.ent_slot, (const float*)s.val, (const float*)s.label, (const float*)c->cW,   \
-                               (const float*)c->cV, s.pred, s.sumvx, (float*)nullptr, f->G, f->Ghot, f->GS, c->cfg.l2_reg, rb, re, hdr, \
-                               c->stat_partial, c->stat_done, out_slot, stats, wf, nw, ep, c->dz, (float*)nullptr);              \
+                               (const uint32_t*)s.ent_slot, (const float*)s.val, (const float*)s.label, c->cW, c->cV, s.pred,  \
+                               s.sumvx, (float*)nullptr, f->G, f->Ghot, f->GS, c->cfg.l2_reg, rb, re, hdr,                      \
+                               c->stat_partial, c->stat_done, out_slot, stats, wf, nw, ep, c->dz, (float*)nullptr, CompactUpd{}); \
         }                                                                                                                        \
     } while (0)
     if (s.has_val) FUSED_LAUNCH(true); else FUSED_LAUNCH(false);
@@ -185,6 +186,52 @@
 int launch_fm_fused(lctr_ctx* c, Slot& s, int64_t rb, int64_t re, bool stats, const int64_t* hdr, double* out_slot_override) {
     return launch_fused_mode(c, s, rb, re, stats, hdr, out_slot_override, 1, PROF_FM_FUSED);
 }
+template <int K, bool HV>
+static cudaError_t fm_step_go(lctr_ctx* c, Slot& s, int64_t rb, int64_t re, double* out_slot, const int64_t* hdr,
+                              const OptParams& P, const OptParams* P_dev) {
+    FusedState* f = c->fused;
+    const auto kern = fm_fused_kernel<K, HV, 1, false, 4, true>;
+    int& grid = f->step_grid[HV ? 1 : 0];
+    if (!grid) {
+        int per_sm = 0;
+        const cudaError_t e = cudaOccupancyMaxActiveBlocksPerMultiprocessor(&per_sm, kern, 128, 0);
+        if (e != cudaSuccess) return e;
+        grid = per_sm * c->sm_count;
+    }
+    const CompactUpd u{s.uniq, s.n_uniq, s.hot_of, s.hot_slot, s.n_hot, c->s1W, c->s1V, c->s2W, c->s2V, P, P_dev};
+    cudaLaunchConfig_t cfg = {};
+    cfg.gridDim = dim3((unsigned)grid); cfg.blockDim = dim3(128); cfg.stream = c->stream;
+    cudaLaunchAttribute at[1];
+    at[0].id = cudaLaunchAttributeCooperative;
+    at[0].val.cooperative = 1;
+    cfg.attrs = at; cfg.numAttrs = 1;
+    return cudaLaunchKernelEx(&cfg, kern, (const int64_t*)s.row_ptr, (const uint32_t*)s.fid, (const uint32_t*)s.ent_slot,
+                              (const float*)s.val, (const float*)s.label, c->W, c->V, s.pred, s.sumvx, (float*)nullptr, f->G,
+                              f->Ghot, f->GS, c->cfg.l2_reg, rb, re, hdr, c->stat_partial, c->stat_done, out_slot, 1,
+                              (const unsigned long long*)nullptr, 0, 0ull, (float*)nullptr, (float*)nullptr, u);
+}
+
+int launch_fm_step(lctr_ctx* c, Slot& s, int64_t rb, int64_t re, const int64_t* hdr, double* out_slot_override,
+                   const OptParams* P_host, const OptParams* dP) {
+    LCTR_CHECK(s.fused_valid, "fused FM step on a slot without its slot map (uploaded before the context supported it?)");
+    const OptParams P = P_host ? *P_host : make_opt_params(c, re - rb);
+    double* out_slot = out_slot_override ? out_slot_override : c->stats + 2 * (c->step % kStatRing);
+    ProfScope prof(c, PROF_FM_FUSED);
+    cudaError_t e;
+#define STEP_GO(KK) (s.has_val ? fm_step_go<KK, true>(c, s, rb, re, out_slot, hdr, P, dP) : fm_step_go<KK, false>(c, s, rb, re, out_slot, hdr, P, dP))
+    switch ((int)c->cfg.factor_cnt) {
+        case 4: e = STEP_GO(4); break;
+        case 8: e = STEP_GO(8); break;
+        case 16: e = STEP_GO(16); break;
+        default: e = STEP_GO(32); break;
+    }
+#undef STEP_GO
+    c->launches++;
+    LCTR_CUDA(e);
+    LCTR_CHECK(c->fused->step_grid[s.has_val ? 1 : 0] > 0, "fused FM step: the kernel fits no CTA on an SM");
+    return 0;
+}
+
 int launch_nfm_forward_fused(lctr_ctx* c, Slot& s, int64_t rb, int64_t re) {
     return launch_fused_mode(c, s, rb, re, false, nullptr, nullptr, 2, PROF_FM_FWD);
 }
@@ -218,22 +265,26 @@
 }
 
 template <int K>
-static void apply_go(lctr_ctx* c, Slot& s, const OptParams& P, const OptParams* P_dev) {
-    FusedState* f = c->fused;
-    const int main_blocks = c->sm_count * 3;
-    const unsigned grid = (unsigned)(main_blocks + kHotMax / 8);
-    const bool pdl_off = !pdl_on();
+static void apply_go(lctr_ctx* c, Slot& s, const OptParams& P) {
+    FusedState* f = c->fused;
     cudaLaunchConfig_t cfg = {};
-    cfg.gridDim = dim3(grid); cfg.blockDim = dim3(256); cfg.dynamicSmemBytes = 0; cfg.stream = c->stream;
+    cfg.blockDim = dim3(256); cfg.dynamicSmemBytes = 0; cfg.stream = c->stream;
     cudaLaunchAttribute attr[1];
     attr[0].id = cudaLaunchAttributeProgrammaticStreamSerialization;
     attr[0].val.programmaticStreamSerializationAllowed = 1;
     cfg.attrs = attr;
-    cfg.numAttrs = (c->cfg.world == 1 && !pdl_off) ? 1 : 0;
+    cfg.numAttrs = (c->cfg.world == 1 && pdl_on()) ? 1 : 0;
+    const CompactUpd u{s.uniq, s.n_uniq, s.hot_of, s.hot_slot, s.n_hot, c->s1W, c->s1V, c->s2W, c->s2V, P, nullptr};
 #define AC_GO(OPTC)                                                                                                          \
-    cudaLaunchKernelEx(&cfg, apply_compact_kernel<K, OPTC>, (const uint32_t*)s.uniq, (const unsigned int*)s.n_uniq, f->G,          \
-                       (const uint32_t*)s.hot_of, (const uint32_t*)s.hot_slot, (const unsigned int*)s.n_hot, f->Ghot, f->GS,     \
-                       main_blocks, c->W, c->V, c->s1W, c->s1V, c->s2W, c->s2V, P, P_dev)
+    do {                                                                                                                     \
+        if (!f->apply_grid) {                                                                                                \
+            int per_sm = 0;                                                                                                  \
+            cudaOccupancyMaxActiveBlocksPerMultiprocessor(&per_sm, apply_compact_kernel<K, OPTC>, 256, 0);                   \
+            f->apply_grid = std::max(1, per_sm) * c->sm_count;                                                               \
+        }                                                                                                                    \
+        cfg.gridDim = dim3((unsigned)f->apply_grid);                                                                         \
+        cudaLaunchKernelEx(&cfg, apply_compact_kernel<K, OPTC>, u, c->W, c->V, f->G, f->Ghot, f->GS);                        \
+    } while (0)
     switch (P.opt) {
         case LCTR_OPT_ADAGRAD: AC_GO(LCTR_OPT_ADAGRAD); break;
         case LCTR_OPT_FTRL: AC_GO(LCTR_OPT_FTRL); break;
@@ -248,14 +299,14 @@
 #undef AC_GO
 }
 
-int launch_apply_compact(lctr_ctx* c, Slot& s, int64_t rows_in_step, const OptParams* P_host, const OptParams* dP) {
-    const OptParams P = P_host ? *P_host : make_opt_params(c, rows_in_step);
+int launch_apply_compact(lctr_ctx* c, Slot& s, int64_t rows_in_step) {
+    const OptParams P = make_opt_params(c, rows_in_step);
     ProfScope prof(c, PROF_APPLY_COMPACT);
     switch ((int)c->cfg.factor_cnt) {
-        case 4: apply_go<4>(c, s, P, dP); break;
-        case 8: apply_go<8>(c, s, P, dP); break;
-        case 16: apply_go<16>(c, s, P, dP); break;
-        default: apply_go<32>(c, s, P, dP); break;
+        case 4: apply_go<4>(c, s, P); break;
+        case 8: apply_go<8>(c, s, P); break;
+        case 16: apply_go<16>(c, s, P); break;
+        default: apply_go<32>(c, s, P); break;
     }
     c->launches++;
     LCTR_CUDA(cudaGetLastError());
diff --git a/lightctr_b200/csrc/fm_fused.cuh b/lightctr_b200/csrc/fm_fused.cuh
--- a/lightctr_b200/csrc/fm_fused.cuh
+++ b/lightctr_b200/csrc/fm_fused.cuh
@@ -1,4 +1,6 @@
 #pragma once
+#include <cooperative_groups.h>
+
 #include "opt.cuh"
 
 namespace lctr {
@@ -147,18 +149,220 @@
     }
 }
 
-template <int K, bool HAS_VAL, int MODE, bool SAME_IDX, int MINB = 4>
+template <int OPT>
+constexpr bool kTwoStates = OPT == LCTR_OPT_FTRL || OPT == LCTR_OPT_ADAM || OPT == LCTR_OPT_ADADELTA || OPT == LCTR_OPT_PS_DCASGD ||
+                            OPT == LCTR_OPT_PS_DCASGDA;
+
+struct CompactUpd {
+    const uint32_t* uniq;
+    const unsigned int* n_uniq;
+    const uint32_t* hot_of;
+    const uint32_t* hot_slot;
+    const unsigned int* n_hot;
+    float *s1W, *s1V, *s2W, *s2V;
+    OptParams P;
+    const OptParams* P_dev;
+};
+
+template <int K>
+struct HotItem {
+    static constexpr int NP = K / 32 + 1;
+    unsigned h;
+    uint32_t f;
+    float wv[NP], av[NP], bv[NP];
+};
+
+template <int K, int OPT>
+__device__ __forceinline__ void hot_load(HotItem<K>& it, unsigned h, const CompactUpd& u, const float* W, const float* V, int GS) {
+    const int lane = threadIdx.x & 31;
+    it.h = h;
+    it.f = __ldg(u.uniq + __ldg(u.hot_slot + h));
+#pragma unroll
+    for (int p = 0; p < HotItem<K>::NP; p++) {
+        const int ncol = GS < 32 ? GS : 32;
+        const int col = 32 * p + lane % ncol;
+        const bool mine = lane / ncol == 0 && col <= K;
+        const size_t o = col < K ? (size_t)it.f * K + col : (size_t)it.f;
+        it.wv[p] = it.av[p] = it.bv[p] = 0.f;
+        if (mine) {
+            it.wv[p] = col < K ? V[o] : W[o];
+            it.av[p] = col < K ? u.s1V[o] : u.s1W[o];
+            if (kTwoStates<OPT>) it.bv[p] = col < K ? u.s2V[o] : u.s2W[o];
+        }
+    }
+}
+
+template <int K, int OPT>
+__device__ __forceinline__ void hot_finish(HotItem<K>& it, const OptParams& P, const CompactUpd& u, float* W, float* V, float* Ghot,
+                                           int GS) {
+    const int lane = threadIdx.x & 31;
+    float* tile = Ghot + (size_t)it.h * kHotRep * GS;
+#pragma unroll
+    for (int p = 0; p < HotItem<K>::NP; p++) {
+        const int ncol = GS < 32 ? GS : 32;
+        const int col = 32 * p + lane % ncol;
+        const int grp = lane / ncol, ngrp = 32 / ncol;
+        const bool mine = grp == 0 && col <= K;
+        const size_t o = col < K ? (size_t)it.f * K + col : (size_t)it.f;
+        float t[kHotRep];
+#pragma unroll
+        for (int i = 0; i < kHotRep; i++)
+            t[i] = (i < kHotRep / ngrp) ? __ldcg(tile + (size_t)(grp + i * ngrp) * GS + col) : 0.f;
+        float sum = 0.f;
+#pragma unroll
+        for (int i = 0; i < kHotRep; i++) {
+            sum += t[i];
+            if (i < kHotRep / ngrp) tile[(size_t)(grp + i * ngrp) * GS + col] = 0.f;
+        }
+        for (int o2 = ncol; o2 < 32; o2 <<= 1) sum += __shfl_xor_sync(kFull, sum, o2);
+        if (mine) {
+            update_one(P, col < K ? P.corrV : P.corrW, it.wv[p], sum, it.av[p], it.bv[p]);
+            if (col < K) { V[o] = it.wv[p]; u.s1V[o] = it.av[p]; if (kTwoStates<OPT>) u.s2V[o] = it.bv[p]; }
+            else { W[o] = it.wv[p]; u.s1W[o] = it.av[p]; if (kTwoStates<OPT>) u.s2W[o] = it.bv[p]; }
+        }
+    }
+}
+
+template <int K>
+struct SlotRows {
+    static constexpr int LPR = K / 4, GR = 32 / LPR, U = 2, N = GR * U;
+    unsigned b0;
+    uint32_t f[U];
+    bool ok[U];
+    float4 v4[U], a4[U], b4[U];
+    float w[U], a[U], bb[U];
+};
+
+template <int K, int OPT>
+__device__ __forceinline__ void rows_load(SlotRows<K>& r, unsigned b0, unsigned total, const CompactUpd& u, const float* W,
+                                          const float* V) {
+    using R = SlotRows<K>;
+    const int lane = threadIdx.x & 31, q = lane % R::LPR, g = lane / R::LPR;
+    r.b0 = b0;
+#pragma unroll
+    for (int i = 0; i < R::U; i++) {
+        const unsigned idx = b0 + i * R::GR + g;
+        r.ok[i] = idx < total && !(u.hot_of && __ldg(u.hot_of + idx) != 0xffffffffu);
+        r.f[i] = r.ok[i] ? __ldg(u.uniq + idx) : 0u;
+        r.v4[i] = r.a4[i] = r.b4[i] = make_float4(0.f, 0.f, 0.f, 0.f);
+        r.w[i] = r.a[i] = r.bb[i] = 0.f;
+        if (r.ok[i]) {
+            const size_t o = (size_t)r.f[i] * K + 4 * q;
+            r.v4[i] = *reinterpret_cast<const float4*>(V + o);
+            r.a4[i] = *reinterpret_cast<const float4*>(u.s1V + o);
+            if (kTwoStates<OPT>) r.b4[i] = *reinterpret_cast<const float4*>(u.s2V + o);
+            if (q == 0) {
+                r.w[i] = W[r.f[i]]; r.a[i] = u.s1W[r.f[i]];
+                if (kTwoStates<OPT>) r.bb[i] = u.s2W[r.f[i]];
+            }
+        }
+    }
+}
+
+template <int K, int OPT>
+__device__ __forceinline__ void rows_finish(SlotRows<K>& r, const OptParams& P, const CompactUpd& u, float* W, float* V, float* G,
+                                            int GS) {
+    using R = SlotRows<K>;
+    const int lane = threadIdx.x & 31, q = lane % R::LPR, g = lane / R::LPR;
+    float4 g4[R::U];
+    float gw[R::U];
+#pragma unroll
+    for (int i = 0; i < R::U; i++) {
+        g4[i] = make_float4(0.f, 0.f, 0.f, 0.f);
+        gw[i] = 0.f;
+        if (r.ok[i]) {
+            const float* grow = G + (size_t)(r.b0 + i * R::GR + g) * GS;
+            g4[i] = __ldcg(reinterpret_cast<const float4*>(grow + 4 * q));
+            if (q == 0) gw[i] = __ldcg(grow + K);
+        }
+    }
+#pragma unroll
+    for (int i = 0; i < R::U; i++) {
+        if (!r.ok[i]) continue;
+        float* grow = G + (size_t)(r.b0 + i * R::GR + g) * GS;
+        const size_t o = (size_t)r.f[i] * K + 4 * q;
+        update_one(P, P.corrV, r.v4[i].x, g4[i].x, r.a4[i].x, r.b4[i].x);
+        update_one(P, P.corrV, r.v4[i].y, g4[i].y, r.a4[i].y, r.b4[i].y);
+        update_one(P, P.corrV, r.v4[i].z, g4[i].z, r.a4[i].z, r.b4[i].z);
+        update_one(P, P.corrV, r.v4[i].w, g4[i].w, r.a4[i].w, r.b4[i].w);
+        *reinterpret_cast<float4*>(V + o) = r.v4[i];
+        *reinterpret_cast<float4*>(u.s1V + o) = r.a4[i];
+        if (kTwoStates<OPT>) *reinterpret_cast<float4*>(u.s2V + o) = r.b4[i];
+        *reinterpret_cast<float4*>(grow + 4 * q) = make_float4(0.f, 0.f, 0.f, 0.f);
+        if (q == 0) {
+            update_one(P, P.corrW, r.w[i], gw[i], r.a[i], r.bb[i]);
+            W[r.f[i]] = r.w[i]; u.s1W[r.f[i]] = r.a[i];
+            if (kTwoStates<OPT>) u.s2W[r.f[i]] = r.bb[i];
+            grow[K] = 0.f;
+        }
+    }
+}
+
+template <int K, int OPT, typename Wait>
+__device__ __forceinline__ void compact_update(const CompactUpd& u, float* W, float* V, float* G, float* Ghot, int GS, unsigned warp,
+                                               unsigned nwarps, Wait wait) {
+    using R = SlotRows<K>;
+    OptParams P = u.P_dev ? *u.P_dev : u.P;
+    P.opt = OPT;
+    const unsigned nh = min(*u.n_hot, (unsigned)kHotMax), total = *u.n_uniq;
+    HotItem<K> hi;
+    R r;
+    if (warp < nh) hot_load<K, OPT>(hi, warp, u, W, V, GS);
+    rows_load<K, OPT>(r, warp * R::N, total, u, W, V);
+    wait();
+    rows_finish<K, OPT>(r, P, u, W, V, G, GS);
+    if (warp < nh) hot_finish<K, OPT>(hi, P, u, W, V, Ghot, GS);
+    for (unsigned h = warp + nwarps; h < nh; h += nwarps) {
+        hot_load<K, OPT>(hi, h, u, W, V, GS);
+        hot_finish<K, OPT>(hi, P, u, W, V, Ghot, GS);
+    }
+    for (unsigned b0 = (warp + nwarps) * R::N; b0 < total; b0 += nwarps * R::N) {
+        rows_load<K, OPT>(r, b0, total, u, W, V);
+        rows_finish<K, OPT>(r, P, u, W, V, G, GS);
+    }
+}
+
+__device__ __forceinline__ void prefetch_l2(const void* p) { asm volatile("prefetch.global.L2 [%0];" ::"l"(p)); }
+
+template <int K>
+__device__ __forceinline__ void prefetch_param_rows(const CompactUpd& u, const float* W, uint32_t f) {
+    prefetch_l2(W + f);
+    prefetch_l2(u.s1W + f);
+    prefetch_l2(u.s1V + (size_t)f * K);
+    if (u.s2V) {
+        prefetch_l2(u.s2W + f);
+        prefetch_l2(u.s2V + (size_t)f * K);
+    }
+}
+
+template <int K>
+__device__ __forceinline__ void compact_prefetch(const CompactUpd& u, const float* W, unsigned warp, unsigned nwarps) {
+    constexpr int N = SlotRows<K>::N;
+    const int lane = threadIdx.x & 31;
+    const unsigned total = __ldg(u.n_uniq), nh = min(__ldg(u.n_hot), (unsigned)kHotMax);
+    if (lane == 0)
+        for (unsigned h = warp; h < nh; h += nwarps) prefetch_param_rows<K>(u, W, __ldg(u.uniq + __ldg(u.hot_slot + h)));
+    for (unsigned b0 = warp * N; b0 < total; b0 += nwarps * N)
+        for (int i = lane; i < N; i += 32) {
+            const unsigned idx = b0 + i;
+            if (idx >= total) continue;
+            const uint32_t f = __ldg(u.uniq + idx);
+            if (!(u.hot_of && __ldg(u.hot_of + idx) != 0xffffffffu)) prefetch_param_rows<K>(u, W, f);
+        }
+}
+
+template <int K, bool HAS_VAL, int MODE, bool SAME_IDX, int MINB = 4, bool UPD = false>
 __global__ void __launch_bounds__(128, MINB)
 fm_fused_kernel(const int64_t* __restrict__ row_ptr, const uint32_t* __restrict__ pidx, const uint32_t* __restrict__ gidx,
-                const float* __restrict__ val, const float* __restrict__ label, const float* __restrict__ W,
-                const float* __restrict__ V, float* __restrict__ pred, float* __restrict__ sumvx, float* __restrict__ dvec,
+                const float* __restrict__ val, const float* __restrict__ label, float* W, float* V, float* __restrict__ pred, float* __restrict__ sumvx, float* __restrict__ dvec,
                 float* __restrict__ G, float* __restrict__ Ghot, int GS, float l2, int64_t rb, int64_t re_arg,
                 const int64_t* __restrict__ hdr, double* partial, unsigned int* done, double* out_slot, int do_stats,
                 const unsigned long long* wait_flags = nullptr, int n_wait = 0, unsigned long long wait_epoch = 0,
                 float* __restrict__ zbuf = nullptr ,
-                float* __restrict__ wide = nullptr ) {
+                float* __restrict__ wide = nullptr , CompactUpd upd = CompactUpd{}) {
     constexpr bool FWD = MODE != 3, BWD = MODE == 1 || MODE == 3, NFM = MODE >= 2;
     static_assert(K % 4 == 0 && K <= 32 && (K / 4 & (K / 4 - 1)) == 0, "fused FM step: K in {4, 8, 16, 32}");
+    static_assert(!UPD || MODE == 1, "the updater tail belongs to the FM step");
     cudaTriggerProgrammaticLaunchCompletion();
     if (wait_flags) {
         if (threadIdx.x < n_wait) {
@@ -178,6 +382,7 @@
     const int64_t gwarp = (int64_t)blockIdx.x * (blockDim.x >> 5) + (threadIdx.x >> 5);
     const int rep = (int)(gwarp & (kHotRep - 1));
     double loss = 0.0, correct = 0.0;
+    if constexpr (UPD) compact_prefetch<K>(upd, W, (unsigned)gwarp, (unsigned)NW);
 
     for (int64_t c0 = rb + gwarp; c0 < re; c0 += 32 * NW) {
         const int64_t myr = c0 + (int64_t)lane * NW;
@@ -398,123 +603,29 @@
         }
     }
     if (do_stats) publish_stats(loss, correct, partial, done, out_slot, false);
+    if constexpr (UPD) {
+        const auto barrier = [] { cooperative_groups::this_grid().sync(); };
+        const unsigned w = (unsigned)gwarp, nw = (unsigned)NW;
+        switch (upd.P.opt) {
+            case LCTR_OPT_ADAGRAD: compact_update<K, LCTR_OPT_ADAGRAD>(upd, W, V, G, Ghot, GS, w, nw, barrier); break;
+            case LCTR_OPT_FTRL: compact_update<K, LCTR_OPT_FTRL>(upd, W, V, G, Ghot, GS, w, nw, barrier); break;
+            case LCTR_OPT_ADAM: compact_update<K, LCTR_OPT_ADAM>(upd, W, V, G, Ghot, GS, w, nw, barrier); break;
+            case LCTR_OPT_RMSPROP: compact_update<K, LCTR_OPT_RMSPROP>(upd, W, V, G, Ghot, GS, w, nw, barrier); break;
+            case LCTR_OPT_ADADELTA: compact_update<K, LCTR_OPT_ADADELTA>(upd, W, V, G, Ghot, GS, w, nw, barrier); break;
+            case LCTR_OPT_PS_SGD: compact_update<K, LCTR_OPT_PS_SGD>(upd, W, V, G, Ghot, GS, w, nw, barrier); break;
+            case LCTR_OPT_PS_ADAGRAD: compact_update<K, LCTR_OPT_PS_ADAGRAD>(upd, W, V, G, Ghot, GS, w, nw, barrier); break;
+            case LCTR_OPT_PS_DCASGD: compact_update<K, LCTR_OPT_PS_DCASGD>(upd, W, V, G, Ghot, GS, w, nw, barrier); break;
+            default: compact_update<K, LCTR_OPT_PS_DCASGDA>(upd, W, V, G, Ghot, GS, w, nw, barrier); break;
+        }
+    }
 }
 
 template <int K, int OPT>
 __global__ void __launch_bounds__(256, 3)
-apply_compact_kernel(const uint32_t* __restrict__ uniq, const unsigned int* __restrict__ n_uniq, float* __restrict__ G,
-                     const uint32_t* __restrict__ hot_of, const uint32_t* __restrict__ hot_slot,
-                     const unsigned int* __restrict__ n_hot, float* __restrict__ Ghot, int GS, int main_blocks,
-                     float* __restrict__ W, float* __restrict__ V, float* __restrict__ s1W, float* __restrict__ s1V,
-                     float* __restrict__ s2W, float* __restrict__ s2V, OptParams P_in, const OptParams* __restrict__ P_dev) {
-    constexpr int LPR = K / 4, GR = 32 / LPR, U = 2;
-    OptParams P = P_dev ? *P_dev : P_in;
-    P.opt = OPT;
-    constexpr bool two = OPT == LCTR_OPT_FTRL || OPT == LCTR_OPT_ADAM || OPT == LCTR_OPT_ADADELTA || OPT == LCTR_OPT_PS_DCASGD ||
-                         OPT == LCTR_OPT_PS_DCASGDA;
-    const int lane = threadIdx.x & 31;
-    if ((int)blockIdx.x >= main_blocks) {
-        const unsigned hwarp = (blockIdx.x - main_blocks) * (blockDim.x >> 5) + (threadIdx.x >> 5);
-        const unsigned nhw = (gridDim.x - main_blocks) * (blockDim.x >> 5);
-        const unsigned nh = min(*n_hot, (unsigned)kHotMax);
-        for (unsigned h = hwarp; h < nh; h += nhw) {
-            const uint32_t slot = __ldg(hot_slot + h);
-            const uint32_t f = __ldg(uniq + slot);
-            float* tile = Ghot + (size_t)h * kHotRep * GS;
-#pragma unroll
-            for (int c0 = 0; c0 < K + 1; c0 += 32) {
-                const int ncol = GS < 32 ? GS : 32;
-                const int col = c0 + lane % ncol;
-                const int grp = lane / ncol, ngrp = 32 / ncol;
-                float wv = 0.f, av = 0.f, bv = 0.f;
-                const bool mine = grp == 0 && col <= K;
-                const size_t o = col < K ? (size_t)f * K + col : (size_t)f;
-                if (mine) {
-                    wv = col < K ? V[o] : W[o];
-                    av = col < K ? s1V[o] : s1W[o];
-                    if (two) bv = col < K ? s2V[o] : s2W[o];
-                }
-                cudaGridDependencySynchronize();
-                float t[kHotRep];
-#pragma unroll
-                for (int i = 0; i < kHotRep; i++)
-                    t[i] = (i < kHotRep / ngrp) ? __ldcg(tile + (size_t)(grp + i * ngrp) * GS + col) : 0.f;
-                float sum = 0.f;
-#pragma unroll
-                for (int i = 0; i < kHotRep; i++) {
-                    sum += t[i];
-                    if (i < kHotRep / ngrp) tile[(size_t)(grp + i * ngrp) * GS + col] = 0.f;
-                }
-                for (int o2 = ncol; o2 < 32; o2 <<= 1) sum += __shfl_xor_sync(kFull, sum, o2);
-                if (mine) {
-                    update_one(P, col < K ? P.corrV : P.corrW, wv, sum, av, bv);
-                    if (col < K) { V[o] = wv; s1V[o] = av; if (two) s2V[o] = bv; }
-                    else { W[o] = wv; s1W[o] = av; if (two) s2W[o] = bv; }
-                }
-            }
-        }
-        cudaGridDependencySynchronize();
-        return;
-    }
-    const unsigned warp = blockIdx.x * (blockDim.x >> 5) + (threadIdx.x >> 5);
-    const unsigned nwarps = (unsigned)main_blocks * (blockDim.x >> 5);
-    const int q = lane % LPR, g = lane / LPR;
-    const unsigned total = *n_uniq;
-    for (unsigned b0 = warp * (GR * U); b0 < total; b0 += nwarps * (GR * U)) {
-        uint32_t f[U];
-        bool ok[U];
-        float4 g4[U], v4[U], a4[U], b4[U];
-        float gw[U], w[U], a[U], bb[U];
-#pragma unroll
-        for (int u = 0; u < U; u++) {
-            const unsigned idx = b0 + u * GR + g;
-            ok[u] = idx < total && !(hot_of && __ldg(hot_of + idx) != 0xffffffffu);
-            f[u] = ok[u] ? __ldg(uniq + idx) : 0u;
-            g4[u] = v4[u] = a4[u] = b4[u] = make_float4(0.f, 0.f, 0.f, 0.f);
-            gw[u] = w[u] = a[u] = bb[u] = 0.f;
-            if (ok[u]) {
-                const size_t o = (size_t)f[u] * K + 4 * q;
-                v4[u] = *reinterpret_cast<const float4*>(V + o);
-                a4[u] = *reinterpret_cast<const float4*>(s1V + o);
-                if (two) b4[u] = *reinterpret_cast<const float4*>(s2V + o);
-                if (q == 0) {
-                    w[u] = W[f[u]]; a[u] = s1W[f[u]];
-                    if (two) bb[u] = s2W[f[u]];
-                }
-            }
-        }
-        cudaGridDependencySynchronize();
-#pragma unroll
-        for (int u = 0; u < U; u++) {
-            if (ok[u]) {
-                const float* grow = G + (size_t)(b0 + u * GR + g) * GS;
-                g4[u] = *reinterpret_cast<const float4*>(grow + 4 * q);
-                if (q == 0) gw[u] = grow[K];
-            }
-        }
-#pragma unroll
-        for (int u = 0; u < U; u++) {
-            if (!ok[u]) continue;
-            const unsigned idx = b0 + u * GR + g;
-            float* grow = G + (size_t)idx * GS;
-            const size_t o = (size_t)f[u] * K + 4 * q;
-            update_one(P, P.corrV, v4[u].x, g4[u].x, a4[u].x, b4[u].x);
-            update_one(P, P.corrV, v4[u].y, g4[u].y, a4[u].y, b4[u].y);
-            update_one(P, P.corrV, v4[u].z, g4[u].z, a4[u].z, b4[u].z);
-            update_one(P, P.corrV, v4[u].w, g4[u].w, a4[u].w, b4[u].w);
-            *reinterpret_cast<float4*>(V + o) = v4[u];
-            *reinterpret_cast<float4*>(s1V + o) = a4[u];
-            if (two) *reinterpret_cast<float4*>(s2V + o) = b4[u];
-            *reinterpret_cast<float4*>(grow + 4 * q) = make_float4(0.f, 0.f, 0.f, 0.f);
-            if (q == 0) {
-                update_one(P, P.corrW, w[u], gw[u], a[u], bb[u]);
-                W[f[u]] = w[u]; s1W[f[u]] = a[u];
-                if (two) s2W[f[u]] = bb[u];
-                grow[K] = 0.f;
-            }
-        }
-    }
-    cudaGridDependencySynchronize();
-}
-
-}
+apply_compact_kernel(CompactUpd u, float* __restrict__ W, float* __restrict__ V, float* __restrict__ G, float* __restrict__ Ghot,
+                     int GS) {
+    compact_update<K, OPT>(u, W, V, G, Ghot, GS, blockIdx.x * (blockDim.x >> 5) + (threadIdx.x >> 5), gridDim.x * (blockDim.x >> 5),
+                           [] { cudaGridDependencySynchronize(); });
+}
+
+}
```

After: 84.61 million, median of 6. 26.0% lower.
